# violetdenim/c3dgs

Hardware: AMD Instinct MI355X
Metric: raster views/sec fwd+bwd @1920x1080 (higher is better)
Workload: dtype f32; 1 GPU; BASELINE.json configs[2]: synth-v1 3M Gaussians, SH deg 3, indexed-camera rasterizer (QAT inner loop), mark_visible+fwd+bwd, 1 view/step/GPU; gaussians=3000000, width=1920, height=1080, sh_codebook=304096, gaussian_codebook=754096, parallelism=replicas x1

## Files before the change

__graft_entry__.py:

```python
import os
import subprocess
import sys

ROOT = os.path.dirname(os.path.abspath(__file__))
if ROOT not in sys.path:
    sys.path.insert(0, ROOT)


def build() -> None:
    from c3dgs_amd import build as hip_build
    lib = hip_build.build()
    assert os.path.exists(lib)
    for variant in hip_build.VARIANTS:
        assert os.path.exists(hip_build.build_variant(variant))
    subprocess.check_call(["make", "-C", os.path.join(ROOT, "oracle"), "-s"])
    import c3dgs_amd
    from c3dgs_amd import _lib
    L = _lib.lib()
    assert L.c3dgs_abi_version() == 4


def smoke() -> None:
    import numpy as np
    import torch
    from tests import cases, gpu_util, synth
    from oracle import oracle as orc

    assert torch.cuda.is_available(), "smoke() needs a GPU"
    torch.cuda.set_device(0)
    for name in ("base", "indexed"):
        inp, cam, indexed = cases.make_case(name)
        st = cases.oracle_forward(inp, cam)
        fw = gpu_util.hip_forward(inp, cam, indexed)
        u = gpu_util.unpack(fw)
        np.testing.assert_array_equal(u["radii"], st.radii)
        np.testing.assert_array_equal(u["keys_sorted"], st.keys_sorted)
        np.testing.assert_array_equal(u["point_list"], st.point_list)
        assert gpu_util.psnr(u["out_color"], st.out_color) >= 80.0
        dL = synth.grad_image(cam["W"], cam["H"]).numpy()
        ref = orc.rasterize_backward(st, dL)
        got = gpu_util.hip_backward(fw, dL)
        for k, v in got.items():
            if ref[k].shape == v.shape and v.size:
                err = gpu_util.rel_inf(v, ref[k])
                assert err <= 1e-4, (name, k, err)
    import c3dgs_amd
    g = torch.Generator().manual_seed(0)
    x = (torch.randn(4096, 48, generator=g) * 0.1).float()
    cb = (torch.randn(512, 48, generator=g) * 0.1).float()
    d, i = c3dgs_amd.weightedDistance(x.cuda(), cb.cuda())
    d_ref, i_ref = orc.weighted_distance(x.numpy(), cb.numpy())
    np.testing.assert_array_equal(i.cpu().numpy(), i_ref)
    np.testing.assert_array_equal(d.cpu().numpy().view(np.uint32), d_ref.view(np.uint32))
    print("smoke ok")


if __name__ == "__main__":
    build()
    if "--smoke" in sys.argv:
        smoke()
```

c3dgs_amd/build.py:

```python
import os
import subprocess
import sys
from concurrent.futures import ThreadPoolExecutor

HERE = os.path.dirname(os.path.abspath(__file__))
CSRC = os.path.join(HERE, "csrc")
OBJ = os.path.join(HERE, "build")
LIB = os.path.join(HERE, "libc3dgs_hip.so")
HIPCC = os.environ.get("HIPCC", "/opt/rocm/bin/hipcc")
ARCH = "gfx950"

COMMON = ["--offload-arch=" + ARCH, "-O3", "-fPIC", "-std=c++17", "-Wall", "-Wno-unused-function",
          "-fno-gpu-rdc", "-DNDEBUG"]
SOURCES = {
    "c_abi.hip": [],
    "c_abi_debug.hip": [],
    "preprocess.hip": ["-ffp-contract=off"],
    "backward_preprocess.hip": ["-ffp-contract=off"] + os.environ.get("C3DGS_BWDPRE_FLAGS", "").split(),
    "binning.hip": [],
    "radix_sort.hip": os.environ.get("C3DGS_SORT_FLAGS", "").split(),
    "render.hip": os.environ.get("C3DGS_RENDER_FLAGS", "-fno-slp-vectorize").split(),
    "vq.hip": ["-mllvm", "-amdgpu-mfma-vgpr-form"] + os.environ.get("C3DGS_VQ_FLAGS", "").split(),
    "draws.hip": [],
    "loss.hip": [],
    "metrics.hip": [],
    "encode.hip": [],
    "knn.hip": ["-ffp-contract=off"],
    "adam.hip": ["-ffp-contract=off"],
    "qat.hip": ["-ffp-contract=off"],
    "densify.hip": ["-ffp-contract=off"],
}
HEADERS = [os.path.join(CSRC, "common.hpp"), os.path.join(CSRC, "gsmath.hpp"), os.path.join(CSRC, "render_diag.hpp"),
           os.path.join(HERE, "..", "include", "c3dgs_hip.h"), os.path.join(HERE, "..", "include", "c3dgs_hip_debug.h")]


def _stale(target, deps):
    if not os.path.exists(target):
        return True
    t = os.path.getmtime(target)
    return any(os.path.getmtime(d) > t for d in deps)


def _compile(name, extra, verbose):
    src = os.path.join(CSRC, name)
    obj = os.path.join(OBJ, name.replace(".hip", ".o"))
    cmd = [HIPCC] + COMMON + extra + ["-c", src, "-o", obj]
    if verbose:
        print(" ".join(cmd), flush=True)
    subprocess.check_call(cmd)
    return obj


VARIANTS = {"spin1": {"radix_sort.hip": ["-DC3DGS_OS_SPIN_LIMIT=1u"]}}
def _diag(mode):
    return {src: ["-DC3DGS_DIAG", mode] for src in ("render.hip", "radix_sort.hip", "diag.hip")}


DIAG_VARIANTS = {"lanes": _diag("-DC3DGS_COUNT_LANES"), "bwdtime": _diag("-DC3DGS_BWD_TIMING"), "ostime": _diag("-DC3DGS_OS_TIMING")}


def build_variant(name, verbose=False):
    build(verbose=verbose)
    flags = {**VARIANTS, **DIAG_VARIANTS}[name]
    odir = os.path.join(HERE, "build", "variant_" + name)
    os.makedirs(odir, exist_ok=True)
    lib = os.path.join(HERE, f"libc3dgs_hip_{name}.so")
    objs, rebuilt = [], False
    for src in list(SOURCES) + [f for f in flags if f not in SOURCES]:
        extra = SOURCES.get(src, [])
        obj = os.path.join(OBJ, src.replace(".hip", ".o"))
        if src in flags:
            obj = os.path.join(odir, src.replace(".hip", ".o"))
            if _stale(obj, [os.path.join(CSRC, src)] + HEADERS + [os.path.abspath(__file__)]):
                cmd = [HIPCC] + COMMON + extra + flags[src] + ["-c", os.path.join(CSRC, src), "-o", obj]
                if verbose:
                    print(" ".join(cmd), flush=True)
                subprocess.check_call(cmd)
                rebuilt = True
        objs.append(obj)
    if rebuilt or _stale(lib, objs):
        subprocess.check_call([HIPCC, "--offload-arch=" + ARCH, "-shared", "-fPIC", "-o", lib] + objs)
    return lib


def build(force=False, verbose=False):
    os.makedirs(OBJ, exist_ok=True)
    deps_common = HEADERS + [os.path.abspath(__file__)]
    todo, objs = [], []
    for name, extra in SOURCES.items():
        obj = os.path.join(OBJ, name.replace(".hip", ".o"))
        objs.append(obj)
        if force or _stale(obj, [os.path.join(CSRC, name)] + deps_common):
            todo.append((name, extra))
    if todo:
        with ThreadPoolExecutor(max_workers=min(4, len(todo))) as ex:
            list(ex.map(lambda t: _compile(t[0], t[1], verbose), todo))
    if force or todo or _stale(LIB, objs):
        cmd = [HIPCC, "--offload-arch=" + ARCH, "-shared", "-fPIC", "-o", LIB] + objs
        if verbose:
            print(" ".join(cmd), flush=True)
        subprocess.check_call(cmd)
    return LIB


if __name__ == "__main__":
    print(build(force="--force" in sys.argv, verbose="--verbose" in sys.argv or "-v" in sys.argv))
    for flag, table in (("--variants", VARIANTS), ("--diag", DIAG_VARIANTS)):
        for v in table if flag in sys.argv else ():
            print(build_variant(v, verbose="--verbose" in sys.argv or "-v" in sys.argv))
```

c3dgs_amd/csrc/binning.hip:

```cpp
#include "common.hpp"
#include <rocprim/device/device_radix_sort.hpp>
#include <rocprim/iterator/counting_iterator.hpp>

namespace c3dgs {

size_t scan_temp_bytes(int P)
{
    size_t a = 0, b = 0;
    (void)rocprim::radix_sort_pairs(nullptr, b, (const uint32_t*)nullptr, (uint32_t*)nullptr, (const uint32_t*)nullptr,
                                    (uint32_t*)nullptr, (size_t)P, 0u, 32u);
    size_t m = a > b ? a : b;
    const size_t os = onesweep_depth_temp_bytes(P);
    if (os > m) m = os;
    return m < 256 ? 256 : m;
}

size_t sort_temp_bytes(int R, int end_bit, int key_bytes)
{
    size_t bytes = 0;
    if (key_bytes == 4)
        (void)rocprim::radix_sort_pairs(nullptr, bytes, (const uint32_t*)nullptr, (uint32_t*)nullptr,
                                        (const uint32_t*)nullptr, (uint32_t*)nullptr, (size_t)R, 0u, (unsigned)end_bit);
    else
        (void)rocprim::radix_sort_pairs(nullptr, bytes, (const uint16_t*)nullptr, (uint16_t*)nullptr,
                                        (const uint32_t*)nullptr, (uint32_t*)nullptr, (size_t)R, 0u, (unsigned)end_bit);
    const size_t os = onesweep_tile_temp_bytes(R, end_bit, key_bytes);
    if (os > bytes) bytes = os;
    const size_t reuse = compact_bin_layout(R).bin_bytes;
    if (reuse > bytes) bytes = reuse;
    return bytes < 256 ? 256 : bytes;
}

__global__ void __launch_bounds__(256)
gather_u64_kernel(int n, const uint32_t* __restrict__ idx, const uint2* __restrict__ src, uint2* __restrict__ dst)
{
    const int i = blockIdx.x * 256 + threadIdx.x;
    if (i < n) dst[i] = src[idx[i]];
}

size_t depth_sort_clear_bytes(int P)
{
    return (onesweep_enabled() && (size_t)P < ((size_t)1 << 30)) ? onesweep_depth_clear_bytes(P) : 0;
}
size_t tile_sort_clear_bytes(int R, int end_bit, int key_bytes)
{
    return (onesweep_enabled() && (size_t)R < ((size_t)1 << 30)) ? onesweep_tile_clear_bytes(R, end_bit, key_bytes) : 0;
}

hipError_t run_depth_sort(void* temp, size_t temp_bytes, const uint32_t* kin, uint32_t* kout, const uint32_t* vin,
                          uint32_t* vout, int P, const uint2* rects, uint2* rects_sorted, hipStream_t s, bool ctrl_cleared,
                          bool rects_fit_bytes)
{
    if (onesweep_enabled() && (size_t)P < ((size_t)1 << 30))
        return onesweep_depth_sort(temp, temp_bytes, kin, kout, vin, vout, P, rects, rects_sorted, s, ctrl_cleared, rects_fit_bytes);
    hipError_t e = vin ? rocprim::radix_sort_pairs(temp, temp_bytes, kin, kout, vin, vout, (size_t)P, 0u, 32u, s)
                       : rocprim::radix_sort_pairs(temp, temp_bytes, kin, kout, rocprim::counting_iterator<uint32_t>(0u), vout,
                                                   (size_t)P, 0u, 32u, s);
    if (e != hipSuccess) return e;
    gather_u64_kernel<<<(P + 255) / 256, 256, 0, s>>>(P, vout, rects, rects_sorted);
    return hipGetLastError();
}

hipError_t run_tile_sort(void* temp, size_t temp_bytes, const void* kin, void* kout, int key_bytes, const uint32_t* vin,
                         uint32_t* vout, int R, int end_bit, hipStream_t s, bool ctrl_cleared)
{
    if (key_bytes == 4) {
        if (onesweep_enabled() && (size_t)R < ((size_t)1 << 30))
            return onesweep_tile_sort32(temp, temp_bytes, (const uint32_t*)kin, (uint32_t*)kout, vin, vout, R, end_bit, s, ctrl_cleared);
        return rocprim::radix_sort_pairs(temp, temp_bytes, (const uint32_t*)kin, (uint32_t*)kout, vin, vout, (size_t)R, 0u, (unsigned)end_bit, s);
    }
    if (onesweep_enabled() && (size_t)R < ((size_t)1 << 30))
        return onesweep_tile_sort(temp, temp_bytes, (const uint16_t*)kin, (uint16_t*)kout, vin, vout, R, end_bit, s, ctrl_cleared);
    return rocprim::radix_sort_pairs(temp, temp_bytes, (const uint16_t*)kin, (uint16_t*)kout, vin, vout, (size_t)R, 0u, (unsigned)end_bit, s);
}

}
```

c3dgs_amd/csrc/c_abi.hip:

```cpp
#include "common.hpp"
#include <cstdlib>
#include <cstring>
#include <mutex>
#include <vector>

namespace c3dgs {

static thread_local std::string g_last_error;
void set_error(const std::string& msg) { g_last_error = msg; }

#define C3DGS_STAGE_TABLE(X)                                                                                                   \
    X(MARK_VISIBLE, "mark_visible") X(PREPROCESS, "preprocess") X(DEPTH_SORT, "depth_sort") X(SCAN, "scan")                    \
    X(DUPLICATE, "duplicate_with_keys") X(SORT, "sort") X(RANGES, "identify_ranges") X(RENDER_FWD, "render_forward")           \
    X(ZERO_PARTIALS, "zero_partials") X(RENDER_BWD, "render_backward") X(BWD_PREPROCESS, "backward_preprocess")                \
    X(WDIST, "weighted_distance") X(VQ_ACC, "vq_accumulate") X(VQ_APPLY, "vq_apply") X(LOSS_FWD, "l1_ssim_forward")            \
    X(LOSS_BWD, "l1_ssim_backward") X(QAT_OBSERVE, "qat_observe") X(QAT_CODEBOOKS, "qat_codebooks")                            \
    X(QAT_VISIBLE, "qat_visible") X(QAT_POINTS, "qat_points") X(QAT_POINTS_BWD, "qat_points_backward")                         \
    X(QAT_CODEBOOKS_BWD, "qat_codebooks_backward") X(ADAM, "adam_step") X(KNN_SORT, "knn_sort") X(KNN_BOUNDS, "knn_bounds")    \
    X(KNN_QUERY, "knn_query")
#define C3DGS_X(id, name) ST_##id,
enum Stage { C3DGS_STAGE_TABLE(C3DGS_X) ST_COUNT };
#undef C3DGS_X
#define C3DGS_X(id, name) name,
static const char* const kStageNames[ST_COUNT] = { C3DGS_STAGE_TABLE(C3DGS_X) };
#undef C3DGS_X
struct ProfRec { int stage; hipEvent_t a, b; };
static std::mutex g_prof_mu;
static bool g_prof_on = false;
static int g_prof_only = -1;
static std::vector<ProfRec> g_prof_recs;
static std::vector<hipEvent_t> g_prof_pool;

struct StageTimer {
    bool on; int stage; hipStream_t s; hipEvent_t a{}, b{};
    StageTimer(int stage_, hipStream_t s_) : on(g_prof_on && (g_prof_only < 0 || g_prof_only == stage_)), stage(stage_), s(s_)
    {
        if (!on) return;
        std::lock_guard<std::mutex> lk(g_prof_mu);
        auto get = [&](hipEvent_t& e) {
            if (!g_prof_pool.empty()) { e = g_prof_pool.back(); g_prof_pool.pop_back(); }
            else if (hipEventCreate(&e) != hipSuccess) on = false;
        };
        get(a); get(b);
        if (on) (void)hipEventRecord(a, s);
    }
    ~StageTimer()
    {
        if (!on) return;
        (void)hipEventRecord(b, s);
        std::lock_guard<std::mutex> lk(g_prof_mu);
        g_prof_recs.push_back({ stage, a, b });
    }
};
#define C3DGS_STAGE_CHECK(stage, debug, stream) C3DGS_STAGE(kStageNames[stage], debug, stream)
#define C3DGS_TIMED_STAGE(stage, debug, stream, ...)                                                \
    do {                                                                                            \
        { StageTimer t_(stage, stream); __VA_ARGS__; }                                              \
        C3DGS_STAGE_CHECK(stage, debug, stream);                                                    \
    } while (0)

struct HostRead {
    uint32_t* pinned = nullptr;
    uint32_t* dev = nullptr;
    uint32_t seq = 0;
    hipEvent_t ev{};
    HostRead()
    {
        const char* e = std::getenv("C3DGS_HOST_READ_COPY");
        const bool want_map = !(e && e[0] == '1');
        if (want_map && hipHostMalloc((void**)&pinned, 64, hipHostMallocMapped | hipHostMallocPortable | hipHostMallocCoherent) == hipSuccess) {
            void* d = nullptr;
            if (hipHostGetDevicePointer(&d, pinned, 0) == hipSuccess) dev = (uint32_t*)d;
            std::memset(pinned, 0, 64);
        } else {
            (void)hipGetLastError();
            if (hipHostMalloc((void**)&pinned, 64, hipHostMallocDefault) != hipSuccess) { pinned = nullptr; return; }
        }
        if (hipEventCreateWithFlags(&ev, hipEventDisableTiming) != hipSuccess) { (void)hipHostFree(pinned); pinned = nullptr; dev = nullptr; }
    }
    uint32_t begin()
    {
        if (!dev) return 0u;
        if (++seq == 0u) seq = 1u;
        return seq;
    }
    int copy_words(const uint32_t* src, hipStream_t s)
    {
        C3DGS_HIP_TRY(hipMemcpyAsync(pinned, src, 2 * sizeof(uint32_t), hipMemcpyDeviceToHost, s));
        return C3DGS_OK;
    }
    int queue_copy(const uint32_t* src, hipStream_t s)
    {
        if (dev) return C3DGS_OK;
        if (int rc = copy_words(src, s)) return rc;
        C3DGS_HIP_TRY(hipEventRecord(ev, s));
        return C3DGS_OK;
    }
    int wait(const uint32_t* src, hipStream_t s, uint32_t words[2])
    {
        if (dev) {
            volatile uint32_t* pad = pinned;
            bool seen = false;
            for (long spins = 0; !seen; spins++) {
                seen = __atomic_load_n(&pad[2], __ATOMIC_ACQUIRE) == seq;
                if (!seen && (spins & 0xffff) == 0xffff) {
                    const hipError_t q = hipStreamQuery(s);
                    if (q == hipErrorNotReady) continue;
                    if (q != hipSuccess) return fail(C3DGS_E_HIP, std::string("num_rendered read: ") + hipGetErrorString(q));
                    seen = __atomic_load_n(&pad[2], __ATOMIC_ACQUIRE) == seq;
                    if (!seen) {
                        if (int rc = copy_words(src, s)) return rc;
                        C3DGS_HIP_TRY(hipStreamSynchronize(s));
                        seen = true;
                    }
                }
            }
        } else {
            hipError_t q = hipErrorNotReady;
            for (long spins = 0; spins < 20000000L && (q = hipEventQuery(ev)) == hipErrorNotReady; spins++) { }
            if (q == hipErrorNotReady) q = hipEventSynchronize(ev);
            if (q != hipSuccess) return fail(C3DGS_E_HIP, std::string("num_rendered read: ") + hipGetErrorString(q));
        }
        words[0] = pinned[0]; words[1] = pinned[1];
        return C3DGS_OK;
    }
};
static HostRead& host_read()
{
    static thread_local HostRead h;
    return h;
}

static int validate(const c3dgs_raster_params* p, bool indexed, bool is_backward)
{
    if (!p) return fail(C3DGS_E_INVALID, "params is NULL");
    if (p->P < 0 || p->W <= 0 || p->H <= 0) return fail(C3DGS_E_INVALID, "P, W, H must be non-negative / positive");
    if (p->P == 0) return C3DGS_OK;
    if (!p->means3D) return fail(C3DGS_E_INVALID, "means3D must have dimensions (num_points, 3)");
    if (!p->background || !p->viewmatrix || !p->projmatrix || !p->campos)
        return fail(C3DGS_E_INVALID, "background, viewmatrix, projmatrix and campos are required");
    if (!is_backward && !p->opacities)
        return fail(C3DGS_E_INVALID, "opacities is required");
    if ((p->sh == nullptr) == (p->colors_precomp == nullptr))
        return fail(C3DGS_E_INVALID, "Please provide excatly one of either SHs or precomputed colors!");
    const bool has_sr = p->scales != nullptr && p->rotations != nullptr;
    if ((p->scales != nullptr) != (p->rotations != nullptr) || has_sr == (p->cov3D_precomp != nullptr))
        return fail(C3DGS_E_INVALID, "Please provide exactly one of either scale/rotation pair or precomputed 3D covariance!");
    if (p->sh) {
        if (p->D < 0 || p->D > 3) return fail(C3DGS_E_INVALID, "SH degree must be in [0,3]");
        if (p->M < (p->D + 1) * (p->D + 1)) return fail(C3DGS_E_INVALID, "sh has fewer coefficients than the active degree needs");
    }
    if (indexed) {
        if (p->sh && !p->sh_indices) return fail(C3DGS_E_INVALID, "indexed rasterizer: sh_indices is required with sh");
        if (has_sr && (!p->g_indices || !p->scale_factors))
            return fail(C3DGS_E_INVALID, "indexed rasterizer: g_indices and scale_factors are required with scales/rotations");
    } else if (p->sh_indices || p->g_indices || p->scale_factors) {
        return fail(C3DGS_E_INVALID, "non-indexed rasterizer: sh_indices / g_indices / scale_factors must be NULL");
    }
    if (tiles_x(p->W) > 65535 || tiles_y(p->H) > 65535) return fail(C3DGS_E_INVALID, "image too large for 16-bit tile coordinates");
    if ((unsigned long long)tiles_x(p->W) * tiles_x(p->W) * tiles_y(p->H) >= (1ull << 32))
        return fail(C3DGS_E_INVALID, "image too large: (tiles per row)^2 x (tile rows) must stay below 2^32");
    return C3DGS_OK;
}

static int forward_impl(const c3dgs_raster_params* pp, bool indexed, c3dgs_resize_fn geom_resize, void* geom_user,
                        c3dgs_resize_fn binning_resize, void* binning_user, c3dgs_resize_fn image_resize, void* image_user,
                        float* out_color, int32_t* radii, int32_t* num_rendered, void* stream_)
{
    if (int rc = validate(pp, indexed, false)) return rc;
    if (!out_color || !num_rendered) return fail(C3DGS_E_INVALID, "out_color and num_rendered are required");
    if (!geom_resize || !binning_resize || !image_resize) return fail(C3DGS_E_INVALID, "resize callbacks are required");
    c3dgs_raster_params p = *pp;
    if (!indexed) { p.sh_indices = nullptr; p.g_indices = nullptr; p.scale_factors = nullptr; }
    hipStream_t s = (hipStream_t)stream_;
    const int P = p.P, W = p.W, H = p.H;
    const int gx = tiles_x(W), gy = tiles_y(H);
    *num_rendered = 0;

    ImageLayout IL; image_layout(W, H, &IL);
    void* img_base = image_resize(image_user, IL.total_bytes);
    if (!img_base) return fail(C3DGS_E_ALLOC, "image buffer allocation failed");
    const ImgPtrs img = img_ptrs(img_base, W, H);

    if (P == 0) {
        C3DGS_HIP_TRY(hipMemsetAsync(out_color, 0, (size_t)3 * W * H * sizeof(float), s));
        C3DGS_HIP_TRY(hipMemsetAsync(img_base, 0, IL.total_bytes, s));
        return C3DGS_OK;
    }
    if (!radii) return fail(C3DGS_E_INVALID, "radii is required");

    c3dgs_geom_layout GL; geom_layout(P, &GL);
    void* geom_base = geom_resize(geom_user, GL.total_bytes + geom_gtab_bytes(p));
    if (!geom_base) return fail(C3DGS_E_ALLOC, "geometry buffer allocation failed");
    const GeomPtrs g = geom_ptrs(geom_base, P);

    uint32_t* sort_err = onesweep_error_word();
    if (!sort_err) return fail(C3DGS_E_HIP, "cannot resolve the sort error word");
    HostRead& hr = host_read();
    if (!hr.pinned) return fail(C3DGS_E_HIP, "pinned host buffer allocation failed");
    const uint32_t host_seq = hr.begin();
    const size_t dclear = depth_sort_clear_bytes(P) <= g.scan_temp_bytes ? depth_sort_clear_bytes(P) : 0;
    { StageTimer t_(ST_PREPROCESS, s);
      if (geom_gtab_bytes(p)) launch_pack_codebook(p, g.gtab, s);
      launch_preprocess(p, g, radii, img.ranges, sort_err, g.scan_temp, dclear / 16, hr.dev, host_seq, s); }
    C3DGS_STAGE_CHECK(ST_PREPROCESS, p.debug, s);
    const uint32_t* r_words = g.block_base + (P + 255) / 256;
    if (int rc = hr.queue_copy(r_words, s)) return rc;
    { StageTimer t_(ST_DEPTH_SORT, s);
      C3DGS_HIP_TRY(run_depth_sort(g.scan_temp, g.scan_temp_bytes, g.depth_keys, g.depth_keys_sorted, nullptr, g.depth_order, P,
                                   reinterpret_cast<const uint2*>(g.rects), g.sorted_offsets, s, dclear != 0,
                                   gx <= 255 && gy <= 255)); }
    C3DGS_STAGE_CHECK(ST_DEPTH_SORT, p.debug, s);
    if (p.debug && onesweep_timed_out(s)) return fail(C3DGS_E_HIP, "depth sort: look-back timed out");
    C3DGS_TIMED_STAGE(ST_SCAN, p.debug, s, launch_depth_order_scan(P, g, s));
    uint32_t words[2];
    if (int rc = hr.wait(r_words, s, words)) return rc;
    const uint32_t R_u = words[0];
    if (words[1] != 0) {
        C3DGS_HIP_TRY(hipMemsetAsync(sort_err, 0, sizeof(uint32_t), s));
        return fail(C3DGS_E_HIP, "radix sort look-back timed out in an earlier rasterizer call on this device: that call's "
                                 "image is NaN and its gradients are invalid (flag cleared, this call was not run)");
    }
    if (R_u > 0x7fffffffu) return fail(C3DGS_E_INVALID, "num_rendered overflows int32");
    const int R = (int)R_u;
    *num_rendered = R;

    c3dgs_binning_layout BL; binning_layout(R, W, H, &BL);
    void* bin_base = binning_resize(binning_user, BL.total_bytes);
    if (!bin_base) return fail(C3DGS_E_ALLOC, "binning buffer allocation failed");
    const BinPtrs b = bin_ptrs(bin_base, R, W, H);

    if (R > 0) {
        const int end_bit = tile_sort_end_bit(W, H);
        size_t tclear = tile_sort_clear_bytes(R, end_bit, b.key_bytes);
        if (tclear > b.sort_temp_bytes) tclear = 0;
        C3DGS_TIMED_STAGE(ST_DUPLICATE, p.debug, s, launch_duplicate_with_keys(P, g, b, gx, sort_err, b.sort_temp, tclear / 16, s));
        { StageTimer t_(ST_SORT, s);
          C3DGS_HIP_TRY(run_tile_sort(b.sort_temp, b.sort_temp_bytes, b.keys_unsorted, b.keys_sorted, b.key_bytes, b.values_unsorted,
                                      b.point_list, R, end_bit, s, tclear != 0)); }
        C3DGS_STAGE_CHECK(ST_SORT, p.debug, s);
        if (p.debug && onesweep_timed_out(s)) return fail(C3DGS_E_HIP, "tile sort: look-back timed out");
        C3DGS_TIMED_STAGE(ST_RANGES, p.debug, s, launch_identify_ranges(R, b.keys_sorted, b.key_bytes, img.ranges, sort_err, s));
    }
    C3DGS_TIMED_STAGE(ST_RENDER_FWD, p.debug, s,
                      launch_render_forward(W, H, img, b.point_list, g.splat, p.background, out_color, compact_ptrs(b, R), sort_err, s));
    return C3DGS_OK;
}

static int backward_impl(const c3dgs_raster_params* pp, bool indexed, const int32_t* radii, const void* geom_buffer,
                         const void* binning_buffer, const void* image_buffer, int32_t R, const float* dL_dout_color,
                         c3dgs_resize_fn ws_resize, void* ws_user, const c3dgs_raster_grads* grads, void* stream_)
{
    if (int rc = validate(pp, indexed, true)) return rc;
    if (!grads) return fail(C3DGS_E_INVALID, "grads is NULL");
    c3dgs_raster_params p = *pp;
    if (!indexed) { p.sh_indices = nullptr; p.g_indices = nullptr; p.scale_factors = nullptr; }
    hipStream_t s = (hipStream_t)stream_;
    const int P = p.P, W = p.W, H = p.H;

    void* cb_zero = nullptr;
    size_t cb_zero16 = 0;
    if (indexed) {
        const size_t n_sh = (grads->dL_dsh && p.sh) ? (size_t)p.SHS * p.M * 3 * sizeof(float) : 0;
        const size_t n_rot = (grads->dL_drotations && p.scales) ? (size_t)p.GS * 4 * sizeof(float) : 0;
        const size_t n_sc = (grads->dL_dscales && p.scales) ? (size_t)p.GS * 3 * sizeof(float) : 0;
        char* a_sh = (char*)grads->dL_dsh; char* a_rot = (char*)grads->dL_drotations; char* a_sc = (char*)grads->dL_dscales;
        if (n_sh && n_rot && n_sc && a_rot == a_sh + n_sh && a_sc == a_rot + n_rot) {
            const size_t n = n_sh + n_rot + n_sc;
            if (p.P > 0 && R >= 0 && ((uintptr_t)a_sh & 15u) == 0) {
                cb_zero = a_sh; cb_zero16 = n / 16;
                if (n % 16) C3DGS_HIP_TRY(hipMemsetAsync(a_sh + cb_zero16 * 16, 0, n % 16, s));
            } else {
                C3DGS_HIP_TRY(hipMemsetAsync(a_sh, 0, n, s));
            }
        } else {
            if (n_sh) C3DGS_HIP_TRY(hipMemsetAsync(a_sh, 0, n_sh, s));
            if (n_sc) C3DGS_HIP_TRY(hipMemsetAsync(a_sc, 0, n_sc, s));
            if (n_rot) C3DGS_HIP_TRY(hipMemsetAsync(a_rot, 0, n_rot, s));
        }
    }
    if (P == 0) return C3DGS_OK;
    if (!radii || !geom_buffer || !image_buffer || !dL_dout_color || (R > 0 && !binning_buffer))
        return fail(C3DGS_E_INVALID, "radii, forward buffers and dL_dout_color are required");
    if (!ws_resize) return fail(C3DGS_E_INVALID, "workspace callback is required");
    if (R < 0) return fail(C3DGS_E_INVALID, "R must be >= 0");

    const GeomPtrs g = geom_ptrs(const_cast<void*>(geom_buffer), P);
    const ImgPtrs img = img_ptrs(const_cast<void*>(image_buffer), W, H);
    void* ws_base = ws_resize(ws_user, c3dgs_backward_workspace_bytes(P, R));
    if (!ws_base) return fail(C3DGS_E_ALLOC, "backward workspace allocation failed");
    const BwdPtrs w = bwd_ptrs(ws_base, P, R);

    { StageTimer t_(ST_ZERO_PARTIALS, s);
      launch_backward_prep(R > 0 ? W : 0, H, img, w.touched, w.touched_bytes / 16, R > 0 ? nullptr : cb_zero, R > 0 ? 0 : cb_zero16, s); }
    if (R > 0) {
        const BinPtrs b = bin_ptrs(const_cast<void*>(binning_buffer), R, W, H);
        C3DGS_TIMED_STAGE(ST_RENDER_BWD, p.debug, s,
                          launch_render_backward(W, H, img, g.splat, g.block_base, p.background, dL_dout_color, w.partials, w.touched,
                                                 compact_ptrs(b, R), cb_zero, cb_zero16, s));
    }
    C3DGS_TIMED_STAGE(ST_BWD_PREPROCESS, p.debug, s, launch_backward_preprocess(p, radii, g, w, *grads, s));
    return C3DGS_OK;
}

}

using namespace c3dgs;

extern "C" {

const char* c3dgs_last_error(void) { return g_last_error.c_str(); }

int c3dgs_profile_enable(int on)
{
    std::lock_guard<std::mutex> lk(g_prof_mu);
    g_prof_on = on != 0;
    return C3DGS_OK;
}

int c3dgs_profile_only(const char* stage_name)
{
    std::lock_guard<std::mutex> lk(g_prof_mu);
    g_prof_only = -1;
    if (!stage_name || !*stage_name) return C3DGS_OK;
    for (int i = 0; i < ST_COUNT; i++)
        if (std::strcmp(stage_name, kStageNames[i]) == 0) { g_prof_only = i; return C3DGS_OK; }
    return fail(C3DGS_E_INVALID, std::string("profile_only: unknown stage ") + stage_name);
}

int c3dgs_profile_read(c3dgs_stage_time* out, int capacity)
{
    std::vector<ProfRec> recs;
    {
        std::lock_guard<std::mutex> lk(g_prof_mu);
        recs.swap(g_prof_recs);
    }
    double total[ST_COUNT] = { 0 };
    long long count[ST_COUNT] = { 0 };
    for (auto& r : recs) {
        float ms = 0.f;
        if (hipEventSynchronize(r.b) == hipSuccess && hipEventElapsedTime(&ms, r.a, r.b) == hipSuccess) {
            total[r.stage] += (double)ms;
            count[r.stage]++;
        }
    }
    {
        std::lock_guard<std::mutex> lk(g_prof_mu);
        for (auto& r : recs) { g_prof_pool.push_back(r.a); g_prof_pool.push_back(r.b); }
    }
    int n = 0;
    for (int i = 0; i < ST_COUNT && n < capacity; i++) {
        if (!count[i]) continue;
        std::memset(&out[n], 0, sizeof(out[n]));
        std::strncpy(out[n].name, kStageNames[i], sizeof(out[n].name) - 1);
        out[n].total_ms = total[i];
        out[n].count = count[i];
        n++;
    }
    return n;
}
int c3dgs_abi_version(void) { return C3DGS_ABI_VERSION; }

int c3dgs_get_geom_layout(int32_t P, c3dgs_geom_layout* out)
{
    if (!out || P < 0) return fail(C3DGS_E_INVALID, "bad arguments");
    geom_layout(P, out);
    return C3DGS_OK;
}
int c3dgs_get_binning_layout(int32_t R, int32_t W, int32_t H, c3dgs_binning_layout* out)
{
    if (!out || R < 0 || W <= 0 || H <= 0) return fail(C3DGS_E_INVALID, "bad arguments");
    binning_layout(R, W, H, out);
    return C3DGS_OK;
}
int c3dgs_get_image_layout(int32_t W, int32_t H, c3dgs_image_layout* out)
{
    if (!out || W <= 0 || H <= 0) return fail(C3DGS_E_INVALID, "bad arguments");
    ImageLayout L; image_layout(W, H, &L);
    *out = L;
    return C3DGS_OK;
}
int c3dgs_get_compact_layout(int32_t R, int32_t W, int32_t H, c3dgs_compact_layout* out)
{
    if (!out || R < 0 || W <= 0 || H <= 0) return fail(C3DGS_E_INVALID, "bad arguments");
    c3dgs_binning_layout BL; binning_layout(R, W, H, &BL);
    const CompactBinLayout C = compact_bin_layout(R);
    ImageLayout IL; image_layout(W, H, &IL);
    out->cqm = BL.sort_temp + C.cqm; out->cid = BL.sort_temp + C.cid;
    out->tile_used_c = IL.tile_used_c; out->n_contrib_c = IL.n_contrib_c;
    return C3DGS_OK;
}
int c3dgs_get_backward_layout(int32_t P, int32_t R, c3dgs_backward_layout* out)
{
    if (!out || P < 0 || R < 0) return fail(C3DGS_E_INVALID, "bad arguments");
    backward_layout(P, R, out);
    return C3DGS_OK;
}
size_t c3dgs_backward_workspace_bytes(int32_t P, int32_t R)
{
    c3dgs_backward_layout L; backward_layout(P, R, &L);
    return L.total_bytes;
}

int c3dgs_mark_visible(int32_t P, const float* means3D, const float* viewmatrix, const float* projmatrix, uint8_t* present,
                       void* stream)
{
    (void)projmatrix;
    if (P < 0) return fail(C3DGS_E_INVALID, "P must be >= 0");
    if (P == 0) return C3DGS_OK;
    if (!means3D || !viewmatrix || !present) return fail(C3DGS_E_INVALID, "means3D, viewmatrix and present are required");
    C3DGS_TIMED_STAGE(ST_MARK_VISIBLE, 0, (hipStream_t)stream, launch_mark_visible(P, means3D, viewmatrix, present, (hipStream_t)stream));
    return C3DGS_OK;
}

int c3dgs_mark_visible_pose(int32_t P, const float* means3D, const float* extrinsic_vector, uint8_t* present, void* stream)
{
    if (P < 0) return fail(C3DGS_E_INVALID, "P must be >= 0");
    if (P == 0) return C3DGS_OK;
    if (!means3D || !extrinsic_vector || !present) return fail(C3DGS_E_INVALID, "means3D, extrinsic_vector and present are required");
    C3DGS_TIMED_STAGE(ST_MARK_VISIBLE, 0, (hipStream_t)stream, launch_mark_visible_pose(P, means3D, extrinsic_vector, present, (hipStream_t)stream));
    return C3DGS_OK;
}

int c3dgs_camera_from_pose(const float* extrinsic_vector, float inv_tan_half_fovx, float inv_tan_half_fovy, float* viewmatrix,
                           float* projmatrix, float* campos, void* stream)
{
    if (!extrinsic_vector || !viewmatrix || !projmatrix || !campos) return fail(C3DGS_E_INVALID, "camera_from_pose: NULL pointer");
    launch_camera_from_pose(extrinsic_vector, inv_tan_half_fovx, inv_tan_half_fovy, viewmatrix, projmatrix, campos, (hipStream_t)stream);
    C3DGS_STAGE("camera_from_pose", 0, (hipStream_t)stream);
    return C3DGS_OK;
}

int c3dgs_rasterize_gaussians(const c3dgs_raster_params* p, c3dgs_resize_fn geom_resize, void* geom_user,
                              c3dgs_resize_fn binning_resize, void* binning_user, c3dgs_resize_fn image_resize,
                              void* image_user, float* out_color, int32_t* radii, int32_t* num_rendered, void* stream)
{
    return forward_impl(p, false, geom_resize, geom_user, binning_resize, binning_user, image_resize, image_user, out_color,
                        radii, num_rendered, stream);
}

int c3dgs_rasterize_gaussians_indexed(const c3dgs_raster_params* p, c3dgs_resize_fn geom_resize, void* geom_user,
                                      c3dgs_resize_fn binning_resize, void* binning_user, c3dgs_resize_fn image_resize,
                                      void* image_user, float* out_color, int32_t* radii, int32_t* num_rendered, void* stream)
{
    return forward_impl(p, true, geom_resize, geom_user, binning_resize, binning_user, image_resize, image_user, out_color,
                        radii, num_rendered, stream);
}

int c3dgs_rasterize_gaussians_backward(const c3dgs_raster_params* p, const int32_t* radii, const void* geom_buffer,
                                       const void* binning_buffer, const void* image_buffer, int32_t R,
                                       const float* dL_dout_color, c3dgs_resize_fn workspace_resize, void* workspace_user,
                                       const c3dgs_raster_grads* grads, void* stream)
{
    return backward_impl(p, false, radii, geom_buffer, binning_buffer, image_buffer, R, dL_dout_color, workspace_resize,
                         workspace_user, grads, stream);
}

int c3dgs_rasterize_gaussians_backward_indexed(const c3dgs_raster_params* p, const int32_t* radii, const void* geom_buffer,
                                               const void* binning_buffer, const void* image_buffer, int32_t R,
                                               const float* dL_dout_color, c3dgs_resize_fn workspace_resize,
                                               void* workspace_user, const c3dgs_raster_grads* grads, void* stream)
{
    return backward_impl(p, true, radii, geom_buffer, binning_buffer, image_buffer, R, dL_dout_color, workspace_resize,
                         workspace_user, grads, stream);
}

int c3dgs_weighted_distance(int64_t N, int32_t C, int32_t K, const float* coefs, const int64_t* gather,
                            const float* codebook, float* out_dist, int64_t* out_idx, void* stream)
{
    if (N < 0 || C < 0 || K <= 0) return fail(C3DGS_E_INVALID, "coefs and codebook must have same number of channels");
    if (N == 0) return C3DGS_OK;
    if (!coefs || !codebook || !out_dist || !out_idx) return fail(C3DGS_E_INVALID, "ceofs and codebook must have dimension 2");
    {
        StageTimer t_(ST_WDIST, (hipStream_t)stream);
        if (launch_weighted_distance(N, C, K, coefs, gather, codebook, out_dist, out_idx, (hipStream_t)stream))
            return fail(C3DGS_E_INVALID, "unsupported channel count");
    }
    C3DGS_STAGE_CHECK(ST_WDIST, 0, (hipStream_t)stream);
    return C3DGS_OK;
}

size_t c3dgs_weighted_distance_ws_bytes(int64_t N, int32_t C, int32_t K) { return wd_ws_bytes(N, C, K); }

int c3dgs_weighted_distance_ws(int64_t N, int32_t C, int32_t K, const float* coefs, const int64_t* gather, const float* codebook,
                               float* out_dist, int64_t* out_idx, void* ws, size_t ws_bytes, void* stream)
{
    if (N < 0 || C < 0 || K <= 0) return fail(C3DGS_E_INVALID, "coefs and codebook must have same number of channels");
    if (N == 0) return C3DGS_OK;
    if (!coefs || !codebook || !out_dist || !out_idx) return fail(C3DGS_E_INVALID, "ceofs and codebook must have dimension 2");
    {
        StageTimer t_(ST_WDIST, (hipStream_t)stream);
        if (launch_weighted_distance(N, C, K, coefs, gather, codebook, out_dist, out_idx, (hipStream_t)stream, ws, ws ? ws_bytes : 0))
            return fail(C3DGS_E_INVALID, "unsupported channel count");
    }
    C3DGS_STAGE_CHECK(ST_WDIST, 0, (hipStream_t)stream);
    return C3DGS_OK;
}

int c3dgs_vq_accumulate(int64_t B, int32_t K, int32_t D, const float* x, const float* w, const int64_t* gather,
                        const int64_t* idx, const float* dist, float* S, double* dist_sum, void* stream)
{
    if (B < 0 || K <= 0 || D <= 0) return fail(C3DGS_E_INVALID, "bad sizes");
    if (B == 0) return C3DGS_OK;
    if (!x || !w || !idx || !S) return fail(C3DGS_E_INVALID, "x, w, idx and S are required");
    C3DGS_TIMED_STAGE(ST_VQ_ACC, 0, (hipStream_t)stream, launch_vq_accumulate(B, K, D, x, w, gather, idx, dist, S, dist_sum, (hipStream_t)stream));
    return C3DGS_OK;
}

int c3dgs_vq_sums(int64_t B, int32_t K, int32_t D, const float* x, const float* w, const int64_t* gather,
                  const float* codebook, float* dist, int64_t* idx, float* S, double* dist_sum, void* ws, size_t ws_bytes,
                  void* stream)
{
    if (B < 0 || K <= 0 || D <= 0) return fail(C3DGS_E_INVALID, "bad sizes");
    if (!S || !dist_sum) return fail(C3DGS_E_INVALID, "S and dist_sum are required");
    C3DGS_HIP_TRY(hipMemsetAsync(S, 0, (size_t)K * (D + 1) * sizeof(float), (hipStream_t)stream));
    C3DGS_HIP_TRY(hipMemsetAsync(dist_sum, 0, sizeof(double), (hipStream_t)stream));
    if (B == 0) return C3DGS_OK;
    if (!x || !w || !codebook || !dist || !idx) return fail(C3DGS_E_INVALID, "x, w, codebook, dist and idx are required");
    {
        StageTimer t_(ST_WDIST, (hipStream_t)stream);
        if (launch_weighted_distance(B, K, D, x, gather, codebook, dist, idx, (hipStream_t)stream, ws, ws ? ws_bytes : 0))
            return fail(C3DGS_E_INVALID, "unsupported channel count");
    }
    C3DGS_STAGE_CHECK(ST_WDIST, 0, (hipStream_t)stream);
    return c3dgs_vq_accumulate(B, K, D, x, w, gather, idx, dist, S, dist_sum, stream);
}

int c3dgs_vq_step_supported(int32_t K, int32_t D, const float* x, const float* codebook, const void* ws, size_t ws_bytes)
{
    return (K > 0 && D > 0 && wd_presplit_supported(K, D, x, codebook, ws, ws_bytes)) ? 1 : 0;
}

int c3dgs_vq_step_sums(int32_t step, int64_t B, int32_t K, int32_t D, const float* x, const float* w, const int64_t* gather,
                       const float* codebook, float* dist, int64_t* idx, float* S, double* dist_sum, void* ws, size_t ws_bytes,
                       void* stream)
{
    hipStream_t s = (hipStream_t)stream;
    if (step < 0 || B <= 0 || K <= 0 || D <= 0) return fail(C3DGS_E_INVALID, "vq_step_sums: bad sizes");
    if (!x || !w || !codebook || !dist || !idx || !S || !dist_sum) return fail(C3DGS_E_INVALID, "vq_step_sums: NULL argument");
    if (!wd_presplit_supported(K, D, x, codebook, ws, ws_bytes))
        return fail(C3DGS_E_INVALID, "vq_step_sums: shape / scratch not served by the fused step (see c3dgs_vq_step_supported)");
    if (step == 0) {
        C3DGS_HIP_TRY(hipMemsetAsync(S, 0, (size_t)K * (D + 1) * sizeof(float), s));
        C3DGS_HIP_TRY(hipMemsetAsync(dist_sum, 0, sizeof(double), s));
    }
    {
        StageTimer t_(ST_WDIST, s);
        if (launch_weighted_distance(B, K, D, x, gather, codebook, dist, idx, s, ws, ws_bytes, step == 0 ? -1 : (step & 1)))
            return fail(C3DGS_E_INVALID, "vq_step_sums: unsupported shape");
        if (step == 0) launch_vq_seed_words(K, D, ws, s);
    }
    C3DGS_STAGE_CHECK(ST_WDIST, 0, s);
    C3DGS_TIMED_STAGE(ST_VQ_ACC, 0, s,
                      launch_vq_accumulate(B, K, D, x, w, gather, idx, dist, S, dist_sum, s, vq_next_absmax_word(K, D, ws, step & 1)));
    return C3DGS_OK;
}

int c3dgs_vq_step_apply(int32_t step, int32_t K, int32_t D, float* S, float* codebook, float* entry_importance, float decay,
                        float alpha, float eps, int32_t scale_normalize, void* ws, size_t ws_bytes, void* stream)
{
    if (step < 0 || K <= 0 || D <= 0 || !S || !codebook || !entry_importance) return fail(C3DGS_E_INVALID, "vq_step_apply: bad arguments");
    { StageTimer t_(ST_VQ_APPLY, (hipStream_t)stream);
      if (launch_vq_apply_split(K, D, S, codebook, entry_importance, decay, alpha, eps, scale_normalize, ws, ws_bytes, step & 1, (hipStream_t)stream))
          return fail(C3DGS_E_INVALID, "vq_step_apply: shape / scratch not served by the fused step (see c3dgs_vq_step_supported)"); }
    C3DGS_STAGE_CHECK(ST_VQ_APPLY, 0, (hipStream_t)stream);
    return C3DGS_OK;
}

int c3dgs_vq_apply(int32_t K, int32_t D, const float* S, float* codebook, float* entry_importance, float decay,
                   float alpha, float eps, int32_t scale_normalize, void* stream)
{
    if (K <= 0 || D <= 0 || !S || !codebook || !entry_importance) return fail(C3DGS_E_INVALID, "bad arguments");
    C3DGS_TIMED_STAGE(ST_VQ_APPLY, 0, (hipStream_t)stream,
                      launch_vq_apply(K, D, S, codebook, entry_importance, decay, alpha, eps, scale_normalize, (hipStream_t)stream));
    return C3DGS_OK;
}

size_t c3dgs_morton_workspace_bytes(int32_t P) { return morton_workspace_bytes(P); }

int c3dgs_morton_order(int32_t P, const float* xyz, int64_t* codes, int64_t* order, void* workspace, void* stream)
{
    if (P < 0) return fail(C3DGS_E_INVALID, "P must be >= 0");
    if (P == 0) return C3DGS_OK;
    if (!xyz || !codes || !order || !workspace) return fail(C3DGS_E_INVALID, "morton_order: bad arguments");
    if (run_morton_order(P, xyz, codes, order, workspace, (hipStream_t)stream)) return fail(C3DGS_E_HIP, "morton_order failed");
    C3DGS_STAGE("morton_order", 0, (hipStream_t)stream);
    return C3DGS_OK;
}

size_t c3dgs_knn_workspace_bytes(int32_t P) { return knn_workspace_bytes(P); }

int c3dgs_knn_mean_dist2(int32_t P, const float* xyz, float* out, void* workspace, void* stream)
{
    if (P < 0) return fail(C3DGS_E_INVALID, "knn_mean_dist2: P must be >= 0");
    if (P == 0) return C3DGS_OK;
    if (!xyz || !out || !workspace) return fail(C3DGS_E_INVALID, "knn_mean_dist2: bad arguments");
    hipStream_t s = (hipStream_t)stream;
    { StageTimer t_(ST_KNN_SORT, s);
      if (run_knn_sort(P, xyz, workspace, s)) return fail(C3DGS_E_HIP, "knn_mean_dist2: sort failed"); }
    C3DGS_STAGE_CHECK(ST_KNN_SORT, 0, s);
    C3DGS_TIMED_STAGE(ST_KNN_BOUNDS, 0, s, launch_knn_bounds(P, workspace, s));
    C3DGS_TIMED_STAGE(ST_KNN_QUERY, 0, s, launch_knn_query(P, workspace, out, s));
    return C3DGS_OK;
}

int c3dgs_abs_accumulate(int64_t n, const float* g, float* acc, void* stream)
{
    if (n < 0 || (n > 0 && (!g || !acc))) return fail(C3DGS_E_INVALID, "abs_accumulate: bad arguments");
    launch_abs_accumulate(n, g, acc, (hipStream_t)stream);
    C3DGS_STAGE("abs_accumulate", 0, (hipStream_t)stream);
    return C3DGS_OK;
}

int c3dgs_adam_step(int32_t n_tensors, const c3dgs_adam_tensor* tensors, double beta1, double beta2, double eps, void* stream)
{
    if (n_tensors < 0 || n_tensors > C3DGS_ADAM_MAX_TENSORS) return fail(C3DGS_E_INVALID, "adam_step: between 0 and 16 tensors per call");
    if (n_tensors == 0) return C3DGS_OK;
    if (!tensors) return fail(C3DGS_E_INVALID, "adam_step: tensors is NULL");
    for (int k = 0; k < n_tensors; k++)
        if (tensors[k].n > 0 && (!tensors[k].param || !tensors[k].grad || !tensors[k].exp_avg || !tensors[k].exp_avg_sq))
            return fail(C3DGS_E_INVALID, "adam_step: NULL tensor pointer");
    C3DGS_TIMED_STAGE(ST_ADAM, 0, (hipStream_t)stream, launch_adam(n_tensors, tensors, beta1, beta2, eps, (hipStream_t)stream));
    return C3DGS_OK;
}

static const int kRowsMaxCopies = 250;

int c3dgs_densify_classify(int32_t P, const float* accum, const float* denom, const float* scale_clone, const float* scale_split,
                           const float* scale_prune_self, const float* scale_prune_child, const float* opacity, float max_grad,
                           float dense_extent, float min_opacity, float big_extent, uint8_t* code, void* stream)
{
    if (P < 0) return fail(C3DGS_E_INVALID, "densify_classify: P must be >= 0");
    if (!(max_grad > 0.f)) return fail(C3DGS_E_INVALID, "densify_classify: max_grad must be > 0 (see include/c3dgs_hip.h)");
    if (P == 0) return C3DGS_OK;
    if (!accum || !denom || !scale_clone || !scale_split || !opacity || !code)
        return fail(C3DGS_E_INVALID, "densify_classify: NULL buffer");
    if ((scale_prune_self == nullptr) != (scale_prune_child == nullptr))
        return fail(C3DGS_E_INVALID, "densify_classify: scale_prune_self and scale_prune_child go together");
    launch_densify_classify(P, accum, denom, scale_clone, scale_split, scale_prune_self, scale_prune_child, opacity, max_grad,
                            dense_extent, min_opacity, big_extent, code, (hipStream_t)stream);
    C3DGS_STAGE("densify_classify", 0, (hipStream_t)stream);
    return C3DGS_OK;
}

size_t c3dgs_rows_plan_workspace_bytes(int32_t P) { return rows_plan_workspace_bytes(P); }

int c3dgs_rows_plan(int32_t P, const uint8_t* code, int32_t N, int64_t capacity, int32_t* src, uint8_t* kind, int32_t* draw_row,
                    int32_t* totals, void* workspace, void* stream)
{
    if (P < 0) return fail(C3DGS_E_INVALID, "rows_plan: P must be >= 0");
    if (N < 1 || N > kRowsMaxCopies) return fail(C3DGS_E_INVALID, "rows_plan: N must be between 1 and 250");
    if (capacity < 0) return fail(C3DGS_E_INVALID, "rows_plan: capacity must be >= 0");
    if ((int64_t)P * (2 + N) >= ((int64_t)1 << 31)) return fail(C3DGS_E_INVALID, "rows_plan: P * (2 + N) must fit 31 bits");
    if (!totals) return fail(C3DGS_E_INVALID, "rows_plan: totals is required");
    hipStream_t s = (hipStream_t)stream;
    if (P == 0) { C3DGS_HIP_TRY(hipMemsetAsync(totals, 0, 4 * sizeof(int32_t), s)); return C3DGS_OK; }
    if (!code || !workspace) return fail(C3DGS_E_INVALID, "rows_plan: NULL buffer");
    if (src && (!kind || !draw_row)) return fail(C3DGS_E_INVALID, "rows_plan: src, kind and draw_row go together");
    C3DGS_HIP_TRY(run_rows_plan(P, code, N, capacity, src, kind, draw_row, totals, workspace, s));
    C3DGS_STAGE("rows_plan", 0, s);
    return C3DGS_OK;
}

int c3dgs_rows_apply(int32_t P, int64_t P_new, const int32_t* src, const uint8_t* kind, const int32_t* draw_row, int32_t n_tensors,
                     const c3dgs_rows_tensor* tensors, int32_t N, int64_t n_draws, const float* rotation_raw, const float* std,
                     const float* z, int32_t log_scaling, int32_t half_xyz, void* stream)
{
    if (P < 0 || P_new < 0 || n_draws < 0) return fail(C3DGS_E_INVALID, "rows_apply: sizes must be >= 0");
    if (N < 1 || N > kRowsMaxCopies) return fail(C3DGS_E_INVALID, "rows_apply: N must be between 1 and 250");
    if (n_tensors < 0 || n_tensors > C3DGS_ROWS_MAX_TENSORS) return fail(C3DGS_E_INVALID, "rows_apply: between 0 and 16 tensors per call");
    if (P_new >= ((int64_t)1 << 31)) return fail(C3DGS_E_INVALID, "rows_apply: P_new must fit 31 bits");
    if (P_new == 0 || n_tensors == 0) return C3DGS_OK;
    if (P == 0) return fail(C3DGS_E_INVALID, "rows_apply: P_new > 0 rows cannot come from P = 0");
    if (!src || !kind || !draw_row || !tensors) return fail(C3DGS_E_INVALID, "rows_apply: NULL buffer");
    for (int k = 0; k < n_tensors; k++) {
        const c3dgs_rows_tensor& t = tensors[k];
        if (t.row_floats < 1 || t.row_floats > 4096) return fail(C3DGS_E_INVALID, "rows_apply: row_floats must be between 1 and 4096");
        if (!t.in_param || !t.out_param) return fail(C3DGS_E_INVALID, "rows_apply: NULL tensor pointer");
        const int nm = (t.in_exp_avg != nullptr) + (t.in_exp_avg_sq != nullptr) + (t.out_exp_avg != nullptr) + (t.out_exp_avg_sq != nullptr);
        if (nm != 0 && nm != 4) return fail(C3DGS_E_INVALID, "rows_apply: the four moment pointers go together");
        if (t.role != C3DGS_ROLE_COPY && t.role != C3DGS_ROLE_XYZ && t.role != C3DGS_ROLE_SCALING)
            return fail(C3DGS_E_INVALID, "rows_apply: unknown role");
        if (t.role != C3DGS_ROLE_COPY && t.row_floats != 3) return fail(C3DGS_E_INVALID, "rows_apply: xyz / scaling rows have 3 floats");
        if (t.role != C3DGS_ROLE_COPY && n_draws > 0 && (!std || !z || (t.role == C3DGS_ROLE_XYZ && !rotation_raw)))
            return fail(C3DGS_E_INVALID, "rows_apply: children need rotation_raw, std and z");
    }
    launch_rows_apply(P, P_new, src, kind, draw_row, n_tensors, tensors, N, n_draws, rotation_raw, std, z, log_scaling, half_xyz, (hipStream_t)stream);
    C3DGS_STAGE("rows_apply", 0, (hipStream_t)stream);
    return C3DGS_OK;
}

int c3dgs_densify_stats(int32_t P, const float* grad, const uint8_t* filter, const int32_t* radii, float* accum, float* denom,
                        float* max_radii, void* stream)
{
    if (P < 0) return fail(C3DGS_E_INVALID, "densify_stats: P must be >= 0");
    if (P == 0) return C3DGS_OK;
    if (!grad || !filter || !accum || !denom) return fail(C3DGS_E_INVALID, "densify_stats: NULL buffer");
    if ((radii == nullptr) != (max_radii == nullptr)) return fail(C3DGS_E_INVALID, "densify_stats: radii and max_radii go together");
    launch_densify_stats(P, grad, filter, radii, accum, denom, max_radii, (hipStream_t)stream);
    C3DGS_STAGE("densify_stats", 0, (hipStream_t)stream);
    return C3DGS_OK;
}

int c3dgs_extract_rot_scale(int32_t n, const float* cov6, float* rot, float* scale, void* stream)
{
    if (n < 0) return fail(C3DGS_E_INVALID, "extract_rot_scale: n must be >= 0");
    if (n == 0) return C3DGS_OK;
    if (!cov6 || !rot || !scale || (reinterpret_cast<uintptr_t>(rot) & 15)) return fail(C3DGS_E_INVALID, "extract_rot_scale: bad arguments");
    launch_extract_rot_scale(n, cov6, rot, scale, (hipStream_t)stream);
    C3DGS_STAGE("extract_rot_scale", 0, (hipStream_t)stream);
    return C3DGS_OK;
}

int c3dgs_l1_ssim_forward(int32_t C, int32_t H, int32_t W, const float* img, const float* gt, float* dmaps, double* sums,
                          void* stream)
{
    if (C <= 0 || H <= 0 || W <= 0 || !img || !gt || !sums) return fail(C3DGS_E_INVALID, "l1_ssim_forward: bad arguments");
    hipStream_t s = (hipStream_t)stream;
    C3DGS_HIP_TRY(hipMemsetAsync(sums, 0, 128 * sizeof(double), s));
    const size_t n = (size_t)C * H * W;
    C3DGS_TIMED_STAGE(ST_LOSS_FWD, 0, s,
                      launch_l1_ssim_forward(C, H, W, img, gt, dmaps, dmaps ? dmaps + n : nullptr, dmaps ? dmaps + 2 * n : nullptr, sums, s));
    return C3DGS_OK;
}

int c3dgs_l1_ssim_value(const double* sums, double l1_scale, double ssim_scale, double constant, float* out, void* stream)
{
    if (!sums || !out) return fail(C3DGS_E_INVALID, "l1_ssim_value: bad arguments");
    launch_l1_ssim_value(sums, l1_scale, ssim_scale, constant, out, (hipStream_t)stream);
    C3DGS_STAGE("l1_ssim_value", 0, (hipStream_t)stream);
    return C3DGS_OK;
}

int c3dgs_l1_ssim_backward(int32_t C, int32_t H, int32_t W, const float* img, const float* gt, const float* dmaps,
                           const float* grad_loss, float l1_coeff, float ssim_coeff, float* dL_dimg, void* stream)
{
    if (C <= 0 || H <= 0 || W <= 0 || !img || !gt || !dmaps || !grad_loss || !dL_dimg)
        return fail(C3DGS_E_INVALID, "l1_ssim_backward: bad arguments");
    hipStream_t s = (hipStream_t)stream;
    const size_t n = (size_t)C * H * W;
    C3DGS_TIMED_STAGE(ST_LOSS_BWD, 0, s,
                      launch_l1_ssim_backward(C, H, W, img, gt, dmaps, dmaps + n, dmaps + 2 * n, grad_loss, l1_coeff, ssim_coeff, dL_dimg, s));
    return C3DGS_OK;
}

size_t c3dgs_image_metrics_ws_bytes(int32_t N, int32_t C, int32_t H, int32_t W) { return image_metrics_ws_bytes(N, C, H, W); }

int c3dgs_image_metrics(int32_t N, int32_t C, int32_t H, int32_t W, const float* img, const float* gt, void* ws, size_t ws_bytes,
                        double* out, void* stream)
{
    if (N <= 0 || C <= 0 || H <= 0 || W <= 0) return fail(C3DGS_E_INVALID, "image_metrics: N, C, H and W must be positive");
    if (image_metrics_workgroups(N, C, H, W) > IMAGE_METRICS_MAX_WORKGROUPS)
        return fail(C3DGS_E_INVALID, "image_metrics: size overflow (N * C * H * W too large for one call; split the batch)");
    if (!img || !gt || !ws || !out) return fail(C3DGS_E_INVALID, "image_metrics: img, gt, ws and out are required");
    if (reinterpret_cast<uintptr_t>(ws) & 7) return fail(C3DGS_E_INVALID, "image_metrics: ws must be 8-byte aligned");
    const size_t need = image_metrics_ws_bytes(N, C, H, W);
    if (ws_bytes < need)
        return fail(C3DGS_E_INVALID, "image_metrics: ws too small (" + std::to_string(ws_bytes) + " bytes, need " +
                                         std::to_string(need) + ")");
    launch_image_metrics(N, C, H, W, img, gt, (double*)ws, out, (hipStream_t)stream);
    C3DGS_STAGE("image_metrics", 0, (hipStream_t)stream);
    return C3DGS_OK;
}

static int qat_validate(const c3dgs_qat_params* q, const char* who)
{
    if (!q) return fail(C3DGS_E_INVALID, std::string(who) + ": params is NULL");
    if (q->P < 0 || q->GS < 0 || q->SHS < 0 || q->M < 1) return fail(C3DGS_E_INVALID, std::string(who) + ": bad sizes");
    if (!q->state) return fail(C3DGS_E_INVALID, std::string(who) + ": state is required");
    if (q->features_dc && q->M > 1 && !q->features_rest)
        return fail(C3DGS_E_INVALID, std::string(who) + ": features_rest is required with features_dc when M > 1");
    if (reinterpret_cast<uintptr_t>(q->rotation) & 15) return fail(C3DGS_E_INVALID, std::string(who) + ": rotation must be 16-byte aligned");
    return C3DGS_OK;
}
static bool misaligned16(const void* p) { return (reinterpret_cast<uintptr_t>(p) & 15) != 0; }

size_t c3dgs_qat_workspace_bytes(void) { return qat_workspace_bytes(); }
size_t c3dgs_qat_scan_bytes(int32_t P) { return qat_scan_bytes(P); }

int c3dgs_qat_observe(const c3dgs_qat_params* q, void* workspace, void* stream)
{
    if (int rc = qat_validate(q, "qat_observe")) return rc;
    if (!workspace) return fail(C3DGS_E_INVALID, "qat_observe: workspace is required");
    C3DGS_TIMED_STAGE(ST_QAT_OBSERVE, 0, (hipStream_t)stream, launch_qat_observe(*q, workspace, (hipStream_t)stream));
    return C3DGS_OK;
}

int c3dgs_qat_codebooks(const c3dgs_qat_params* q, float* scales_n, float* rotations, float* shs, void* stream)
{
    if (int rc = qat_validate(q, "qat_codebooks")) return rc;
    if (misaligned16(rotations) || misaligned16(shs)) return fail(C3DGS_E_INVALID, "qat_codebooks: outputs must be 16-byte aligned");
    C3DGS_TIMED_STAGE(ST_QAT_CODEBOOKS, 0, (hipStream_t)stream, launch_qat_codebooks(*q, scales_n, rotations, shs, (hipStream_t)stream));
    return C3DGS_OK;
}

int c3dgs_qat_codebooks_backward(const c3dgs_qat_params* q, const float* dL_dscales_n, const float* dL_drotations,
                                 const float* dL_dshs, float* dL_dscaling, float* dL_drotation, float* dL_dfeatures_dc,
                                 float* dL_dfeatures_rest, void* stream)
{
    if (int rc = qat_validate(q, "qat_codebooks_backward")) return rc;
    if (misaligned16(dL_drotations) || misaligned16(dL_drotation) || misaligned16(dL_dshs))
        return fail(C3DGS_E_INVALID, "qat_codebooks_backward: rotation / sh gradients must be 16-byte aligned");
    if (dL_dshs && q->features_dc && (!dL_dfeatures_dc || (q->M > 1 && !dL_dfeatures_rest)))
        return fail(C3DGS_E_INVALID, "qat_codebooks_backward: dL_dfeatures_dc / dL_dfeatures_rest are required with dL_dshs");
    C3DGS_TIMED_STAGE(ST_QAT_CODEBOOKS_BWD, 0, (hipStream_t)stream,
                      launch_qat_codebooks_backward(*q, dL_dscales_n, dL_drotations, dL_dshs, dL_dscaling, dL_drotation, dL_dfeatures_dc,
                                                    dL_dfeatures_rest, (hipStream_t)stream));
    return C3DGS_OK;
}

int c3dgs_qat_visible(const c3dgs_qat_params* q, const float* viewmatrix, uint8_t* visible, int32_t* rank, int32_t* count,
                      void* scan_workspace, void* stream)
{
    if (int rc = qat_validate(q, "qat_visible")) return rc;
    if (!count) return fail(C3DGS_E_INVALID, "qat_visible: count is required");
    hipStream_t s = (hipStream_t)stream;
    if (q->P == 0) { C3DGS_HIP_TRY(hipMemsetAsync(count, 0, sizeof(int32_t), s)); return C3DGS_OK; }
    if (!q->xyz || !viewmatrix || !visible || !rank || !scan_workspace) return fail(C3DGS_E_INVALID, "qat_visible: bad arguments");
    { StageTimer t_(ST_QAT_VISIBLE, s); C3DGS_HIP_TRY(run_qat_visible(*q, viewmatrix, visible, rank, count, scan_workspace, s)); }
    C3DGS_STAGE_CHECK(ST_QAT_VISIBLE, 0, s);
    return C3DGS_OK;
}

int c3dgs_qat_points(const c3dgs_qat_params* q, const uint8_t* visible, const int32_t* rank, const int64_t* sh_indices,
                     const int64_t* g_indices, float* means3D, float* opacities, float* scale_factors, int64_t* sh_indices_out,
                     int64_t* g_indices_out, void* stream)
{
    if (int rc = qat_validate(q, "qat_points")) return rc;
    if ((visible == nullptr) != (rank == nullptr)) return fail(C3DGS_E_INVALID, "qat_points: visible and rank go together");
    C3DGS_TIMED_STAGE(ST_QAT_POINTS, 0, (hipStream_t)stream,
                      launch_qat_points(*q, visible, rank, sh_indices, g_indices, means3D, opacities, scale_factors, sh_indices_out,
                                        g_indices_out, (hipStream_t)stream));
    return C3DGS_OK;
}

int c3dgs_qat_points_backward(const c3dgs_qat_params* q, const uint8_t* visible, const int32_t* rank, const float* dL_dmeans3D,
                              const float* dL_dmeans2D, const float* dL_dopacities, const float* dL_dscale_factors,
                              float* dL_dxyz, float* dL_dscreenspace, float* dL_dopacity, float* dL_dscaling_factor, void* stream)
{
    if (int rc = qat_validate(q, "qat_points_backward")) return rc;
    if ((visible == nullptr) != (rank == nullptr)) return fail(C3DGS_E_INVALID, "qat_points_backward: visible and rank go together");
    if ((dL_dopacity && dL_dopacities && !q->opacity) || (dL_dscaling_factor && dL_dscale_factors && !q->scaling_factor))
        return fail(C3DGS_E_INVALID, "qat_points_backward: the raw opacity / scaling_factor are needed to recompute the masks");
    C3DGS_TIMED_STAGE(ST_QAT_POINTS_BWD, 0, (hipStream_t)stream,
                      launch_qat_points_backward(*q, visible, rank, dL_dmeans3D, dL_dmeans2D, dL_dopacities, dL_dscale_factors, dL_dxyz,
                                                 dL_dscreenspace, dL_dopacity, dL_dscaling_factor, (hipStream_t)stream));
    return C3DGS_OK;
}

int c3dgs_qat_quantize(const c3dgs_qat_params* q, int32_t scaling_is_exp, int8_t* opacity, int8_t* scaling, int8_t* scaling_factor,
                       int8_t* rotation, int8_t* features_dc, int8_t* features_rest, void* stream)
{
    if (int rc = qat_validate(q, "qat_quantize")) return rc;
    if (rotation && (reinterpret_cast<uintptr_t>(rotation) & 3)) return fail(C3DGS_E_INVALID, "qat_quantize: rotation output must be 4-byte aligned");
    launch_qat_quantize(*q, scaling_is_exp, opacity, scaling, scaling_factor, rotation, features_dc, features_rest, (hipStream_t)stream);
    C3DGS_STAGE("qat_quantize", 0, (hipStream_t)stream);
    return C3DGS_OK;
}

int c3dgs_fake_quantize(int64_t n, const float* x, c3dgs_fq_state* state, int32_t observe, int32_t enabled,
                        float averaging_constant, float* out, void* workspace, void* stream)
{
    if (n < 0) return fail(C3DGS_E_INVALID, "fake_quantize: n must be >= 0");
    if (n == 0) return C3DGS_OK;
    if (!x || !state || !out || (observe && !workspace)) return fail(C3DGS_E_INVALID, "fake_quantize: bad arguments");
    launch_fake_quantize(n, x, state, observe, enabled, averaging_constant, out, workspace, (hipStream_t)stream);
    C3DGS_STAGE("fake_quantize", 0, (hipStream_t)stream);
    return C3DGS_OK;
}

int c3dgs_fake_quantize_backward(int64_t n, const float* x, const c3dgs_fq_state* state, int32_t enabled, const float* g,
                                 float* dx, void* stream)
{
    if (n < 0) return fail(C3DGS_E_INVALID, "fake_quantize_backward: n must be >= 0");
    if (n == 0) return C3DGS_OK;
    if (!x || !state || !g || !dx) return fail(C3DGS_E_INVALID, "fake_quantize_backward: bad arguments");
    launch_fake_quantize_backward(n, x, state, enabled, g, dx, (hipStream_t)stream);
    C3DGS_STAGE("fake_quantize_backward", 0, (hipStream_t)stream);
    return C3DGS_OK;
}

}
```

c3dgs_amd/csrc/common.hpp:

```cpp
#pragma once
#include <hip/hip_runtime.h>
#include <cstdint>
#include <cstddef>
#include <cstdio>
#include <cstring>
#include <string>

#include "../../include/c3dgs_hip.h"

namespace c3dgs {

constexpr int TILE = 16;
constexpr int TILE_PIX = 256;
constexpr int SPLAT_F4 = 3;
constexpr int PARTIAL_FLOATS = 9;
constexpr int BWD_LIST = 1024;

void set_error(const std::string& msg);
inline int fail(int code, const std::string& msg) { set_error(msg); return code; }

#define C3DGS_HIP_TRY(expr)                                                                         \
    do {                                                                                            \
        hipError_t e__ = (expr);                                                                    \
        if (e__ != hipSuccess)                                                                      \
            return ::c3dgs::fail(C3DGS_E_HIP, std::string(#expr) + ": " + hipGetErrorString(e__));  \
    } while (0)

#define C3DGS_STAGE(name, debug, stream)                                                            \
    do {                                                                                            \
        hipError_t e__ = hipGetLastError();                                                         \
        if (e__ == hipSuccess && (debug)) e__ = hipStreamSynchronize(stream);                       \
        if (e__ != hipSuccess)                                                                      \
            return ::c3dgs::fail(C3DGS_E_HIP, std::string("stage ") + name + ": " + hipGetErrorString(e__)); \
    } while (0)

__device__ __forceinline__ uint32_t f2ord(float f)
{
    const uint32_t u = __float_as_uint(f);
    return (u & 0x80000000u) ? ~u : (u | 0x80000000u);
}
__device__ __host__ __forceinline__ float ord2f(uint32_t o)
{
    const uint32_t u = (o & 0x80000000u) ? (o & 0x7fffffffu) : ~o;
    float f;
    memcpy(&f, &u, 4);
    return f;
}

inline size_t align_up(size_t v, size_t a = 256) { return (v + a - 1) / a * a; }

size_t scan_temp_bytes(int P);
size_t sort_temp_bytes(int R, int end_bit, int key_bytes = 2);

inline int tiles_x(int W) { return (W + TILE - 1) / TILE; }
inline int tiles_y(int H) { return (H + TILE - 1) / TILE; }

inline uint32_t higher_msb(uint32_t n)
{
    uint32_t msb = sizeof(n) * 4, step = msb;
    while (step > 1) {
        step /= 2;
        if (n >> msb) msb += step; else msb -= step;
    }
    if (n >> msb) msb++;
    return msb;
}

inline void geom_layout(int P, c3dgs_geom_layout* L)
{
    size_t o = 0, p = (size_t)(P > 0 ? P : 1);
    L->splat = o;             o = align_up(o + p * SPLAT_F4 * 16);
    L->depth_keys = o;        o = align_up(o + p * 4);
    L->depth_keys_sorted = o; o = align_up(o + p * 4);
    L->depth_order = o;       o = align_up(o + p * 4);
    L->sorted_offsets = o;    o = align_up(o + p * 8);
    L->inst_offset = o;       o = align_up(o + p * 4);
    L->rects = o;             o = align_up(o + p * 8);
    L->clamped = o;           o = align_up(o + p);
    L->block_base = o;        o = align_up(o + ((p + 255) / 256 + 2) * 4);
    L->depth_base = o;        o = align_up(o + ((p + 255) / 256 + 1) * 4);
    L->scan_temp = o;         L->scan_temp_bytes = scan_temp_bytes((int)p);
    o = align_up(o + L->scan_temp_bytes);
    L->total_bytes = o;
}

inline size_t geom_gtab_bytes(const c3dgs_raster_params& p) { return (p.g_indices && p.scales) ? align_up((size_t)(p.GS > 0 ? p.GS : 1) * 32) : 0; }

inline int tile_key_bytes_for(long long T) { return T > 65536 ? 4 : 2; }
inline int tile_key_bytes(int W, int H) { return tile_key_bytes_for((long long)tiles_x(W) * tiles_y(H)); }
inline int tile_sort_end_bit_for(long long T)
{
    const int msb = (int)higher_msb((uint32_t)T), kbits = 8 * tile_key_bytes_for(T);
    return msb < kbits ? msb : kbits;
}
inline int tile_sort_end_bit(int W, int H) { return tile_sort_end_bit_for((long long)tiles_x(W) * tiles_y(H)); }

inline void binning_layout(int R, int W, int H, c3dgs_binning_layout* L)
{
    size_t o = 0, r = (size_t)(R > 0 ? R : 1);
    const int end_bit = tile_sort_end_bit(W, H);
    const size_t kb = (size_t)tile_key_bytes(W, H);
    L->keys_unsorted = o;   o = align_up(o + r * kb);
    L->values_unsorted = o; o = align_up(o + r * 4);
    L->keys_sorted = o;     o = align_up(o + r * kb);
    L->point_list = o;      o = align_up(o + r * 4);
    L->sort_temp = o;       L->sort_temp_bytes = sort_temp_bytes((int)r, end_bit, (int)kb);
    o = align_up(o + L->sort_temp_bytes);
    L->total_bytes = o;
}

struct ImageLayout : c3dgs_image_layout { size_t tile_used_c, n_contrib_c; };
inline void image_layout(int W, int H, ImageLayout* L)
{
    size_t o = 0, n = (size_t)W * H, t = (size_t)tiles_x(W) * tiles_y(H);
    L->final_T = o;     o = align_up(o + n * 4);
    L->n_contrib = o;   o = align_up(o + n * 4);
    L->ranges = o;      o = align_up(o + t * 8);
    L->tile_used = o;   o = align_up(o + t * 4);
    L->tile_order = o;  o = align_up(o + t * 4);
    L->tile_used_c = o; o = align_up(o + t * 4);
    L->n_contrib_c = o; o = align_up(o + n * 4);
    L->total_bytes = o;
}

struct CompactBinLayout { size_t cqm, cid, bin_bytes; };
inline CompactBinLayout compact_bin_layout(int R)
{
    const size_t r = (size_t)(R > 0 ? R : 1);
    CompactBinLayout C;
    C.cqm = 0; C.cid = align_up(r); C.bin_bytes = C.cid + align_up(r * 4);
    return C;
}

inline void backward_layout(int P, int R, c3dgs_backward_layout* L)
{
    size_t o = 0, r = (size_t)(R > 0 ? R : 1), n_lists = ((size_t)(P > 0 ? P : 1) + BWD_LIST - 1) / BWD_LIST;
    L->partials = o;   o = align_up(o + r * PARTIAL_FLOATS * sizeof(float));
    L->touched = o;    o = align_up(o + r);
    L->live_ids = o;   o = align_up(o + n_lists * BWD_LIST * 4);
    L->live_slots = o; o = align_up(o + n_lists * BWD_LIST * 4);
    L->live_count = o; o = align_up(o + n_lists * 4);
    L->list_len = BWD_LIST;
    L->total_bytes = o;
}

struct GeomPtrs {
    float4* splat; uint32_t* depth_keys; uint32_t* depth_keys_sorted;
    uint32_t* depth_order; uint2* sorted_offsets; uint32_t* inst_offset; uint16_t* rects;
    uint8_t* clamped; uint32_t* block_base; uint32_t* depth_base; void* scan_temp; size_t scan_temp_bytes;
    float4* gtab;
};
struct BinPtrs {
    void* keys_unsorted; uint32_t* values_unsorted; void* keys_sorted; uint32_t* point_list;
    void* sort_temp; size_t sort_temp_bytes; int key_bytes;
};
struct ImgPtrs { float* final_T; uint32_t* n_contrib; uint2* ranges; uint32_t* tile_used; uint32_t* tile_order;
                 uint32_t* tile_used_c; uint32_t* n_contrib_c; };
struct CompactPtrs { uint8_t* cqm; uint32_t* cid; };
struct BwdPtrs { float* partials; uint8_t* touched; size_t touched_bytes;
                 uint32_t* live_ids; uint32_t* live_slots; uint32_t* live_count; };

inline GeomPtrs geom_ptrs(void* base, int P)
{
    c3dgs_geom_layout L; geom_layout(P, &L);
    char* b = (char*)base;
    return { (float4*)(b + L.splat), (uint32_t*)(b + L.depth_keys), (uint32_t*)(b + L.depth_keys_sorted), (uint32_t*)(b + L.depth_order),
             (uint2*)(b + L.sorted_offsets), (uint32_t*)(b + L.inst_offset), (uint16_t*)(b + L.rects),
             (uint8_t*)(b + L.clamped), (uint32_t*)(b + L.block_base), (uint32_t*)(b + L.depth_base), (void*)(b + L.scan_temp),
             L.scan_temp_bytes, (float4*)(b + L.total_bytes) };
}
inline BinPtrs bin_ptrs(void* base, int R, int W, int H)
{
    c3dgs_binning_layout L; binning_layout(R, W, H, &L);
    char* b = (char*)base;
    return { (void*)(b + L.keys_unsorted), (uint32_t*)(b + L.values_unsorted), (void*)(b + L.keys_sorted),
             (uint32_t*)(b + L.point_list), (void*)(b + L.sort_temp), L.sort_temp_bytes, tile_key_bytes(W, H) };
}
inline ImgPtrs img_ptrs(void* base, int W, int H)
{
    ImageLayout L; image_layout(W, H, &L);
    char* b = (char*)base;
    return { (float*)(b + L.final_T), (uint32_t*)(b + L.n_contrib), (uint2*)(b + L.ranges), (uint32_t*)(b + L.tile_used),
             (uint32_t*)(b + L.tile_order), (uint32_t*)(b + L.tile_used_c), (uint32_t*)(b + L.n_contrib_c) };
}
inline CompactPtrs compact_ptrs(const BinPtrs& bp, int R)
{
    const CompactBinLayout C = compact_bin_layout(R);
    return { (uint8_t*)bp.sort_temp + C.cqm, (uint32_t*)((char*)bp.sort_temp + C.cid) };
}
inline BwdPtrs bwd_ptrs(void* base, int P, int R)
{
    c3dgs_backward_layout L; backward_layout(P, R, &L);
    char* b = (char*)base;
    return { (float*)(b + L.partials), (uint8_t*)(b + L.touched), L.live_ids - L.touched,
             (uint32_t*)(b + L.live_ids), (uint32_t*)(b + L.live_slots), (uint32_t*)(b + L.live_count) };
}

void launch_camera_from_pose(const float* pose, float inv_tan_x, float inv_tan_y, float* view, float* proj, float* campos, hipStream_t s);
void launch_mark_visible(int P, const float* means3D, const float* view, uint8_t* present, hipStream_t s);
void launch_mark_visible_pose(int P, const float* means3D, const float* pose7, uint8_t* present, hipStream_t s);
void launch_pack_codebook(const c3dgs_raster_params& p, float4* gtab, hipStream_t s);
void launch_preprocess(const c3dgs_raster_params& p, const GeomPtrs& g, int32_t* radii, uint2* ranges, const uint32_t* sort_err,
                       void* zero_span, size_t zero_n16, uint32_t* host_out, uint32_t host_seq, hipStream_t s);
void launch_depth_order_scan(int P, const GeomPtrs& g, hipStream_t s);
void launch_duplicate_with_keys(int P, const GeomPtrs& g, const BinPtrs& b, int grid_x, const uint32_t* sort_err,
                                void* zero_span, size_t zero_n16, hipStream_t s);
void launch_identify_ranges(int R, const void* keys_sorted, int key_bytes, uint2* ranges, const uint32_t* sort_err, hipStream_t s);
hipError_t run_depth_sort(void* temp, size_t temp_bytes, const uint32_t* kin, uint32_t* kout, const uint32_t* vin,
                          uint32_t* vout, int P, const uint2* rects, uint2* rects_sorted, hipStream_t s, bool ctrl_cleared = false,
                          bool rects_fit_bytes = false);
hipError_t run_tile_sort(void* temp, size_t temp_bytes, const void* kin, void* kout, int key_bytes, const uint32_t* vin,
                         uint32_t* vout, int R, int end_bit, hipStream_t s, bool ctrl_cleared = false);
size_t depth_sort_clear_bytes(int P);
size_t tile_sort_clear_bytes(int R, int end_bit, int key_bytes);
bool onesweep_enabled();
int onesweep_timed_out(hipStream_t s);
uint32_t* onesweep_error_word();
size_t onesweep_depth_temp_bytes(int P);
size_t onesweep_tile_temp_bytes(int R, int end_bit, int key_bytes = 2);
size_t onesweep_depth_clear_bytes(int P);
size_t onesweep_tile_clear_bytes(int R, int end_bit, int key_bytes);
hipError_t onesweep_depth_sort(void* temp, size_t temp_bytes, const uint32_t* kin, uint32_t* kout, const uint32_t* vin, uint32_t* vout,
                               int P, const uint2* gather_src, uint2* gather_dst, hipStream_t s, bool ctrl_cleared = false,
                               bool rects_fit_bytes = false);
hipError_t onesweep_tile_sort32(void* temp, size_t temp_bytes, const uint32_t* kin, uint32_t* kout, const uint32_t* vin, uint32_t* vout,
                                int R, int end_bit, hipStream_t s, bool ctrl_cleared = false);
hipError_t onesweep_tile_sort(void* temp, size_t temp_bytes, const uint16_t* kin, uint16_t* kout, const uint32_t* vin, uint32_t* vout,
                              int R, int end_bit, hipStream_t s, bool ctrl_cleared = false);
void launch_render_forward(int W, int H, const ImgPtrs& img, const uint32_t* point_list, const float4* splat,
                           const float* bg, float* out_color, const CompactPtrs& cl, const uint32_t* sort_err, hipStream_t s);
void launch_backward_prep(int W, int H, const ImgPtrs& img, void* zero_a, size_t n16_a, void* zero_b, size_t n16_b, hipStream_t s);
void launch_render_backward(int W, int H, const ImgPtrs& img, const float4* splat,
                            const uint32_t* block_base, const float* bg, const float* dL_dpix, float* partials,
                            uint8_t* touched, const CompactPtrs& cl, void* zero_span, size_t zero_n16, hipStream_t s);
void launch_backward_preprocess(const c3dgs_raster_params& p, const int32_t* radii, const GeomPtrs& g, const BwdPtrs& w,
                                const c3dgs_raster_grads& gr, hipStream_t s);
int launch_weighted_distance(int64_t N, int C, int K, const float* coefs, const int64_t* gather, const float* codebook,
                             float* out_dist, int64_t* out_idx, hipStream_t s, void* ws = nullptr, size_t ws_bytes = 0, int presplit = -1);
bool wd_presplit_supported(int C, int K, const float* coefs, const float* codebook, const void* ws, size_t ws_bytes);
int launch_vq_apply_split(int K, int D, float* S, float* codebook, float* entry_importance, float decay, float alpha, float eps,
                          int scale_normalize, void* ws, size_t ws_bytes, int parity, hipStream_t s);
void launch_vq_seed_words(int K, int D, void* ws, hipStream_t s);
uint32_t* vq_next_absmax_word(int K, int D, void* ws, int parity);
size_t wd_ws_bytes(int64_t N, int C, int K);
int launch_wd_debug_scores(int64_t N, int C, int K, const float* coefs, const float* codebook, float* scores, void* ws, size_t ws_bytes,
                           float* out_dist, int64_t* out_idx, hipStream_t s);
void launch_vq_accumulate(int64_t B, int K, int D, const float* x, const float* w, const int64_t* gather,
                          const int64_t* idx, const float* dist, float* S, double* dist_sum, hipStream_t s, uint32_t* clear_word = nullptr);
void launch_vq_apply(int K, int D, const float* S, float* codebook, float* entry_importance, float decay, float alpha,
                     float eps, int scale_normalize, hipStream_t s);

size_t morton_workspace_bytes(int P);
int run_morton_order(int P, const float* xyz, int64_t* codes_out, int64_t* order_out, void* workspace, hipStream_t s);
void launch_extract_rot_scale(int n, const float* cov6, float* rot, float* scale, hipStream_t s);
size_t knn_workspace_bytes(int P);
int run_knn_sort(int P, const float* xyz, void* workspace, hipStream_t s);
void launch_knn_bounds(int P, void* workspace, hipStream_t s);
void launch_knn_query(int P, const void* workspace, float* out, hipStream_t s);
void launch_adam(int n_tensors, const c3dgs_adam_tensor* tensors, double beta1, double beta2, double eps, hipStream_t s);
void launch_abs_accumulate(int64_t n, const float* g, float* acc, hipStream_t s);
void launch_densify_classify(int P, const float* accum, const float* denom, const float* scale_clone, const float* scale_split,
                             const float* scale_prune_self, const float* scale_prune_child, const float* opacity, float max_grad,
                             float dense_extent, float min_opacity, float big_extent, uint8_t* code, hipStream_t s);
size_t rows_plan_workspace_bytes(int P);
hipError_t run_rows_plan(int P, const uint8_t* code, int N, long long capacity, int32_t* src, uint8_t* kind, int32_t* draw_row,
                         int32_t* totals, void* workspace, hipStream_t s);
void launch_rows_apply(int P, long long P_new, const int32_t* src, const uint8_t* kind, const int32_t* draw_row, int n_tensors,
                       const c3dgs_rows_tensor* tensors, int N, long long n_draws, const float* rotation_raw, const float* std,
                       const float* z, int log_scaling, int half_xyz, hipStream_t s);
void launch_densify_stats(int P, const float* grad, const uint8_t* filter, const int32_t* radii, float* accum, float* denom,
                          float* max_radii, hipStream_t s);
void launch_l1_ssim_value(const double* sums, double l1_scale, double ssim_scale, double constant, float* out, hipStream_t s);
void launch_l1_ssim_forward(int C, int H, int W, const float* img, const float* gt, float* Dmu, float* Ds1, float* Ds12,
                            double* sums, hipStream_t s);
void launch_l1_ssim_backward(int C, int H, int W, const float* img, const float* gt, const float* Dmu, const float* Ds1,
                             const float* Ds12, const float* grad_loss, float l1_coeff, float ssim_coeff, float* dL_dimg,
                             hipStream_t s);
constexpr int64_t IMAGE_METRICS_MAX_WORKGROUPS = (int64_t(1) << 24) - 1;
int64_t image_metrics_workgroups(int N, int C, int H, int W);
size_t image_metrics_ws_bytes(int N, int C, int H, int W);
void launch_image_metrics(int N, int C, int H, int W, const float* img, const float* gt, double* partials, double* out,
                          hipStream_t s);

size_t qat_workspace_bytes();
size_t qat_scan_bytes(int P);
void launch_qat_observe(const c3dgs_qat_params& q, void* workspace, hipStream_t s);
void launch_qat_codebooks(const c3dgs_qat_params& q, float* scales_n, float* rotations, float* shs, hipStream_t s);
void launch_qat_codebooks_backward(const c3dgs_qat_params& q, const float* g_scales, const float* g_rot, const float* g_shs,
                                   float* d_scaling, float* d_rotation, float* d_dc, float* d_rest, hipStream_t s);
hipError_t run_qat_visible(const c3dgs_qat_params& q, const float* view, uint8_t* visible, int32_t* rank, int32_t* count,
                           void* scan_ws, hipStream_t s);
void launch_qat_points(const c3dgs_qat_params& q, const uint8_t* visible, const int32_t* rank, const int64_t* sh_idx,
                       const int64_t* g_idx, float* means3D, float* opac, float* sfac, int64_t* sh_out, int64_t* g_out,
                       hipStream_t s);
void launch_qat_points_backward(const c3dgs_qat_params& q, const uint8_t* visible, const int32_t* rank, const float* g_m3,
                                const float* g_m2, const float* g_op, const float* g_sf, float* d_xyz, float* d_screen,
                                float* d_op, float* d_sf, hipStream_t s);
void launch_qat_quantize(const c3dgs_qat_params& q, int scaling_exp, int8_t* opacity, int8_t* scaling, int8_t* scaling_factor,
                         int8_t* rotation, int8_t* features_dc, int8_t* features_rest, hipStream_t s);
void launch_fake_quantize(long long n, const float* x, c3dgs_fq_state* state, int observe, int enabled, float c, float* out,
                          void* workspace, hipStream_t s);
void launch_fake_quantize_backward(long long n, const float* x, const c3dgs_fq_state* state, int enabled, const float* g,
                                   float* dx, hipStream_t s);

}
```

c3dgs_amd/csrc/preprocess.hip:

```cpp
#include "common.hpp"
#include "gsmath.hpp"

namespace c3dgs {

template <bool POSE>
__global__ void __launch_bounds__(256)
mark_visible_kernel(int P, const float* __restrict__ means3D, const float* __restrict__ view_or_pose, uint8_t* __restrict__ present, int vec)
{
    const int j = blockIdx.x * 256 + threadIdx.x;
    const int i0 = 4 * j;
    if (i0 >= P) return;
    float vm[16];
    const float* view = view_or_pose;
    if (POSE) {
        const float x = view_or_pose[0], y = view_or_pose[1], z = view_or_pose[2], w = view_or_pose[3], tz = view_or_pose[6];
        const float d2 = y * y + z * z + x * x;
#pragma unroll
        for (int q = 0; q < 16; q++) vm[q] = 0.f;
        vm[2] = 2.0f * (x * z - w * y); vm[6] = 2.0f * (y * z + w * x); vm[10] = 1.0f + 2.0f * (z * z - d2); vm[14] = tz;
        view = vm;
    }
    if (vec && i0 + 4 <= P) {
        const float4* src = reinterpret_cast<const float4*>(means3D) + 3 * (size_t)j;
        const float4 a = src[0], b = src[1], c = src[2];
        const f3 p0 = { a.x, a.y, a.z }, p1 = { a.w, b.x, b.y }, p2 = { b.z, b.w, c.x }, p3 = { c.y, c.z, c.w };
        const uint32_t v0 = !(xform4x3(p0, view).z <= 0.01f), v1 = !(xform4x3(p1, view).z <= 0.01f);
        const uint32_t v2 = !(xform4x3(p2, view).z <= 0.01f), v3 = !(xform4x3(p3, view).z <= 0.01f);
        reinterpret_cast<uint32_t*>(present)[j] = v0 | (v1 << 8) | (v2 << 16) | (v3 << 24);
        return;
    }
    for (int i = i0; i < min(i0 + 4, P); i++) {
        f3 p = { means3D[3 * (size_t)i], means3D[3 * (size_t)i + 1], means3D[3 * (size_t)i + 2] };
        f3 pv = xform4x3(p, view);
        present[i] = !(pv.z <= 0.01f) ? 1 : 0;
    }
}

__global__ void __launch_bounds__(256)
pack_codebook_kernel(int GS, const float* __restrict__ scales, const float* __restrict__ rotations, float4* __restrict__ gtab)
{
    const int g = blockIdx.x * 256 + threadIdx.x;
    if (g >= GS) return;
    gtab[2 * (size_t)g] = *reinterpret_cast<const float4*>(rotations + 4 * (size_t)g);
    gtab[2 * (size_t)g + 1] = make_float4(scales[3 * (size_t)g], scales[3 * (size_t)g + 1], scales[3 * (size_t)g + 2], 0.f);
}

void launch_pack_codebook(const c3dgs_raster_params& p, float4* gtab, hipStream_t s)
{
    if (p.GS <= 0) return;
    pack_codebook_kernel<<<(p.GS + 255) / 256, 256, 0, s>>>(p.GS, p.scales, p.rotations, gtab);
}

void launch_mark_visible(int P, const float* means3D, const float* view, uint8_t* present, hipStream_t s)
{
    if (P <= 0) return;
    const int vec = ((reinterpret_cast<uintptr_t>(means3D) & 15u) == 0 && (reinterpret_cast<uintptr_t>(present) & 3u) == 0) ? 1 : 0;
    mark_visible_kernel<false><<<((P + 3) / 4 + 255) / 256, 256, 0, s>>>(P, means3D, view, present, vec);
}

void launch_mark_visible_pose(int P, const float* means3D, const float* pose, uint8_t* present, hipStream_t s)
{
    if (P <= 0) return;
    const int vec = ((reinterpret_cast<uintptr_t>(means3D) & 15u) == 0 && (reinterpret_cast<uintptr_t>(present) & 3u) == 0) ? 1 : 0;
    mark_visible_kernel<true><<<((P + 3) / 4 + 255) / 256, 256, 0, s>>>(P, means3D, pose, present, vec);
}

__global__ void camera_from_pose_kernel(const float* __restrict__ pose, float inv_tan_x, float inv_tan_y, float pa, float pb,
                                        float* __restrict__ view, float* __restrict__ proj, float* __restrict__ campos)
{
    if (threadIdx.x != 0 || blockIdx.x != 0) return;
    const float x = pose[0], y = pose[1], z = pose[2], w = pose[3], tx = pose[4], ty = pose[5], tz = pose[6];
    const float d2 = y * y + z * z + x * x;
    float M[4][4];
    M[0][0] = 1.0f + 2.0f * (x * x - d2); M[0][1] = 2.0f * (x * y - w * z);        M[0][2] = 2.0f * (x * z + w * y);        M[0][3] = tx;
    M[1][0] = 2.0f * (x * y + w * z);        M[1][1] = 1.0f + 2.0f * (y * y - d2); M[1][2] = 2.0f * (y * z - w * x);        M[1][3] = ty;
    M[2][0] = 2.0f * (x * z - w * y);        M[2][1] = 2.0f * (y * z + w * x);        M[2][2] = 1.0f + 2.0f * (z * z - d2); M[2][3] = tz;
    M[3][0] = 0.f; M[3][1] = 0.f; M[3][2] = 0.f; M[3][3] = 1.f;
#pragma unroll
    for (int i = 0; i < 4; i++) {
#pragma unroll
        for (int j = 0; j < 4; j++) view[i * 4 + j] = M[j][i];
        proj[i * 4 + 0] = M[0][i] * inv_tan_x;
        proj[i * 4 + 1] = M[1][i] * inv_tan_y;
        proj[i * 4 + 2] = M[2][i] * pa + M[3][i] * pb;
        proj[i * 4 + 3] = M[2][i];
    }
    const double a = M[0][0], b = M[0][1], c = M[0][2], d = M[1][0], e = M[1][1], f = M[1][2], g = M[2][0], h = M[2][1], k = M[2][2];
    const double A = e * k - f * h, B = -(d * k - f * g), C = d * h - e * g;
    const double det = a * A + b * B + c * C;
    const double inv[3][3] = { { A / det, -(b * k - c * h) / det, (b * f - c * e) / det },
                               { B / det, (a * k - c * g) / det, -(a * f - c * d) / det },
                               { C / det, -(a * h - b * g) / det, (a * e - b * d) / det } };
#pragma unroll
    for (int r = 0; r < 3; r++) campos[r] = (float)-(inv[r][0] * (double)tx + inv[r][1] * (double)ty + inv[r][2] * (double)tz);
}

void launch_camera_from_pose(const float* pose, float inv_tan_x, float inv_tan_y, float* view, float* proj, float* campos, hipStream_t s)
{
    const float pa = (float)(1.0 * 100.0 / (100.0 - 0.01)), pb = (float)(-(100.0 * 0.01) / (100.0 - 0.01));
    camera_from_pose_kernel<<<1, 64, 0, s>>>(pose, inv_tan_x, inv_tan_y, pa, pb, view, proj, campos);
}

template <int DEG>
__device__ __forceinline__ void sh_to_rgb(const float* c, float x, float y, float z, float out[3])
{
#pragma unroll
    for (int ch = 0; ch < 3; ch++) {
        float res = SH_C0 * c[0 * 3 + ch];
        if (DEG > 0) {
            res = res - SH_C1 * y * c[1 * 3 + ch] + SH_C1 * z * c[2 * 3 + ch] - SH_C1 * x * c[3 * 3 + ch];
            if (DEG > 1) {
                float xx = x * x, yy = y * y, zz = z * z;
                float xy = x * y, yz = y * z, xz = x * z;
                res = res + SH_C2_0 * xy * c[4 * 3 + ch] + SH_C2_1 * yz * c[5 * 3 + ch] +
                      SH_C2_2 * (2.0f * zz - xx - yy) * c[6 * 3 + ch] + SH_C2_3 * xz * c[7 * 3 + ch] +
                      SH_C2_4 * (xx - yy) * c[8 * 3 + ch];
                if (DEG > 2) {
                    res = res + SH_C3_0 * y * (3.0f * xx - yy) * c[9 * 3 + ch] + SH_C3_1 * xy * z * c[10 * 3 + ch] +
                          SH_C3_2 * y * (4.0f * zz - xx - yy) * c[11 * 3 + ch] +
                          SH_C3_3 * z * (2.0f * zz - 3.0f * xx - 3.0f * yy) * c[12 * 3 + ch] +
                          SH_C3_4 * x * (4.0f * zz - xx - yy) * c[13 * 3 + ch] + SH_C3_5 * z * (xx - yy) * c[14 * 3 + ch] +
                          SH_C3_6 * x * (xx - 3.0f * yy) * c[15 * 3 + ch];
                }
            }
        }
        out[ch] = res + 0.5f;
    }
}

struct PreArgs {
    int P, M, W, H, gx, gy;
    const float* means3D; const float* sh; const float* colors_precomp; const float* opacities;
    const float* scales; const float* scale_factors; const float* rotations; const float* cov3D_precomp;
    const int64_t* sh_indices; const int64_t* g_indices;
    const float* view; const float* proj; const float* campos;
    float tan_fovx, tan_fovy, focal_x, focal_y, scale_modifier;
    int prefiltered, clamp_color;
    int32_t* radii; float4* splat; uint16_t* rects; uint8_t* clamped;
    uint32_t* depth_keys;
    uint32_t* inst_offset; uint32_t* block_total;
    uint2* ranges; int T;
    const float4* gtab;
    uint4* zero_span; size_t zero_n16;
};

template <int DEG>
__global__ void __launch_bounds__(256) preprocess_kernel(const PreArgs a)
{
    __shared__ uint32_t s_wsum[4];
    const int t = threadIdx.x, lane = t & 63, wave = t >> 6;
    const int i = blockIdx.x * 256 + t;
    const bool in_range = i < a.P;
    for (int q = i; q < a.T; q += gridDim.x * 256) a.ranges[q] = make_uint2(0u, 0u);
    if (a.zero_n16) {
        const size_t per = (a.zero_n16 + gridDim.x - 1) / gridDim.x, z0 = (size_t)blockIdx.x * per, z1 = min(z0 + per, a.zero_n16);
        for (size_t q = z0 + t; q < z1; q += 256) a.zero_span[q] = make_uint4(0u, 0u, 0u, 0u);
    }

    int32_t out_radius = 0;
    uint32_t out_tiles = 0;
    uint32_t out_key = 0xffffffffu;
    bool alive = false;
    float4 rec0 = make_float4(0, 0, 0, 0), rec1 = rec0;
    float rgb2 = 0.f;
    uint32_t rect_lo = 0, rect_hi = 0;
    if (in_range) do {
        const f3 p = { a.means3D[3 * (size_t)i], a.means3D[3 * (size_t)i + 1], a.means3D[3 * (size_t)i + 2] };
        const f3 p_view = xform4x3(p, a.view);
        if (!a.prefiltered && p_view.z <= 0.01f) break;

        const float4 p_hom = xform4x4(p, a.proj);
        const float p_w = 1.0f / (p_hom.w + 0.0000001f);
        const float projx = p_hom.x * p_w, projy = p_hom.y * p_w;

        float cov3D[6];
        if (a.cov3D_precomp) {
#pragma unroll
            for (int q = 0; q < 6; q++) cov3D[q] = a.cov3D_precomp[6 * (size_t)i + q];
        } else if (a.g_indices) {
            const size_t g = (size_t)a.g_indices[i];
            const float4 rot = a.gtab[2 * g], sc = a.gtab[2 * g + 1];
            cov3d_from_scale_rot(sc.x, sc.y, sc.z, a.scale_factors[i] * a.scale_modifier, rot, cov3D);
        } else {
            const float4 rot = *reinterpret_cast<const float4*>(a.rotations + 4 * (size_t)i);
            cov3d_from_scale_rot(a.scales[3 * (size_t)i], a.scales[3 * (size_t)i + 1], a.scales[3 * (size_t)i + 2],
                                 a.scale_modifier, rot, cov3D);
        }
        const Cov2D cv = cov2d(p, a.focal_x, a.focal_y, a.tan_fovx, a.tan_fovy, cov3D, a.view);

        const float det = (cv.a * cv.c - cv.b * cv.b);
        if (det == 0.0f) break;
        const float det_inv = 1.f / det;
        const float conic_a = cv.c * det_inv, conic_b = -cv.b * det_inv, conic_c = cv.a * det_inv;

        const float mid = 0.5f * (cv.a + cv.c);
        const float lambda1 = mid + sqrtf(fmaxf(0.1f, mid * mid - det));
        const float lambda2 = mid - sqrtf(fmaxf(0.1f, mid * mid - det));
        const float my_radius = ceilf(3.f * sqrtf(fmaxf(lambda1, lambda2)));
        const float pix = ndc2pix(projx, a.W), piy = ndc2pix(projy, a.H);
        int x0, y0, x1, y1;
        get_rect(pix, piy, (int)my_radius, a.gx, a.gy, x0, y0, x1, y1);
        if ((x1 - x0) * (y1 - y0) == 0) break;

        float rgb[3];
        uint8_t clamp_bits = 0;
        if (a.colors_precomp) {
            rgb[0] = a.colors_precomp[3 * (size_t)i];
            rgb[1] = a.colors_precomp[3 * (size_t)i + 1];
            rgb[2] = a.colors_precomp[3 * (size_t)i + 2];
        } else {
            const size_t row = a.sh_indices ? (size_t)a.sh_indices[i] : (size_t)i;
            const float* shp = a.sh + row * (size_t)a.M * 3;
            constexpr int NC = (DEG + 1) * (DEG + 1) * 3;
            float c[NC];
            if ((a.M * 3) % 4 == 0 && NC % 4 == 0) {
#pragma unroll
                for (int q = 0; q < NC / 4; q++) {
                    const float4 v = reinterpret_cast<const float4*>(shp)[q];
                    c[4 * q] = v.x; c[4 * q + 1] = v.y; c[4 * q + 2] = v.z; c[4 * q + 3] = v.w;
                }
            } else {
#pragma unroll
                for (int q = 0; q < NC; q++) c[q] = shp[q];
            }
            f3 dir = { p.x - a.campos[0], p.y - a.campos[1], p.z - a.campos[2] };
            const float len = sqrtf(dir.x * dir.x + dir.y * dir.y + dir.z * dir.z);
            dir.x = dir.x / len; dir.y = dir.y / len; dir.z = dir.z / len;
            sh_to_rgb<DEG>(c, dir.x, dir.y, dir.z, rgb);
            if (a.clamp_color) {
#pragma unroll
                for (int ch = 0; ch < 3; ch++) {
                    if (rgb[ch] < 0) clamp_bits |= (uint8_t)(1u << ch);
                    rgb[ch] = fmaxf(rgb[ch], 0.0f);
                }
            }
        }

        alive = true;
        out_radius = (int32_t)my_radius;
        out_tiles = (uint32_t)((y1 - y0) * (x1 - x0));
        out_key = __float_as_uint(p_view.z);
        a.clamped[i] = clamp_bits;
        uint16_t* rc = a.rects + 4 * (size_t)i;
        rc[0] = (uint16_t)x0; rc[1] = (uint16_t)y0; rc[2] = (uint16_t)x1; rc[3] = (uint16_t)y1;
        rec0 = make_float4(pix, piy, conic_a, conic_b);
        rec1 = make_float4(conic_c, a.opacities[i], rgb[0], rgb[1]);
        rgb2 = rgb[2];
        rect_lo = (uint32_t)x0 | ((uint32_t)y0 << 16);
        rect_hi = (uint32_t)x1 | ((uint32_t)y1 << 16);
    } while (false);

    uint32_t incl = out_tiles;
#pragma unroll
    for (int o = 1; o < 64; o <<= 1) { const uint32_t v = __shfl_up(incl, o); if (lane >= o) incl += v; }
    if (lane == 63) s_wsum[wave] = incl;
    __syncthreads();
    uint32_t woff = 0;
    for (int w = 0; w < wave; w++) woff += s_wsum[w];
    const uint32_t my_incl = woff + incl;
    if (t == 255) a.block_total[blockIdx.x] = my_incl;
    if (!in_range) return;
    if (!alive) *reinterpret_cast<uint2*>(a.rects + 4 * (size_t)i) = make_uint2(0u, 0u);
    if (alive) {
        float4* rec = a.splat + 3 * (size_t)i;
        rec[0] = rec0;
        rec[1] = rec1;
        rec[2] = make_float4(rgb2, __uint_as_float(my_incl - out_tiles), __uint_as_float(rect_lo), __uint_as_float(rect_hi));
    }
    a.inst_offset[i] = my_incl;
    a.radii[i] = out_radius;
    a.depth_keys[i] = out_key;
}

__global__ void __launch_bounds__(1024) scan_blocks_kernel(int nb, uint32_t* __restrict__ base, const uint32_t* __restrict__ sort_err,
                                                           uint32_t* __restrict__ host_out, uint32_t host_seq)
{
    __shared__ uint32_t s_w[2][16];
    const int t = threadIdx.x, lane = t & 63, wave = t >> 6;
    uint32_t carry = 0;
    int buf = 0;
    for (int c0 = 0; c0 < nb; c0 += 16384, buf ^= 1) {
        const int i0 = c0 + t * 16;
        uint32_t v[16];
#pragma unroll
        for (int q = 0; q < 4; q++) {
            uint4 x = make_uint4(0u, 0u, 0u, 0u);
            if (i0 + 4 * q + 3 < nb) x = reinterpret_cast<const uint4*>(base + i0)[q];
            else {
                if (i0 + 4 * q < nb) x.x = base[i0 + 4 * q];
                if (i0 + 4 * q + 1 < nb) x.y = base[i0 + 4 * q + 1];
                if (i0 + 4 * q + 2 < nb) x.z = base[i0 + 4 * q + 2];
            }
            v[4 * q] = x.x; v[4 * q + 1] = x.y; v[4 * q + 2] = x.z; v[4 * q + 3] = x.w;
        }
        uint32_t mine = 0;
#pragma unroll
        for (int q = 0; q < 16; q++) mine += v[q];
        uint32_t incl = mine;
#pragma unroll
        for (int o = 1; o < 64; o <<= 1) { const uint32_t u = __shfl_up(incl, o); if (lane >= o) incl += u; }
        if (lane == 63) s_w[buf][wave] = incl;
        __syncthreads();
        uint32_t off = carry, all = 0;
#pragma unroll
        for (int w = 0; w < 16; w++) { const uint32_t x = s_w[buf][w]; if (w < wave) off += x; all += x; }
        uint32_t run = off + incl - mine;
#pragma unroll
        for (int q = 0; q < 16; q++) { const uint32_t x = v[q]; v[q] = run; run += x; }
#pragma unroll
        for (int q = 0; q < 4; q++) {
            if (i0 + 4 * q + 3 < nb) reinterpret_cast<uint4*>(base + i0)[q] = make_uint4(v[4 * q], v[4 * q + 1], v[4 * q + 2], v[4 * q + 3]);
            else {
                if (i0 + 4 * q < nb) base[i0 + 4 * q] = v[4 * q];
                if (i0 + 4 * q + 1 < nb) base[i0 + 4 * q + 1] = v[4 * q + 1];
                if (i0 + 4 * q + 2 < nb) base[i0 + 4 * q + 2] = v[4 * q + 2];
            }
        }
        carry += all;
    }
    __syncthreads();
    if (t == 0) {
        base[nb] = carry;
        const uint32_t err = sort_err ? *sort_err : 0u;
        if (sort_err) base[nb + 1] = err;
        if (host_out) {
            __hip_atomic_store(host_out, carry, __ATOMIC_RELAXED, __HIP_MEMORY_SCOPE_SYSTEM);
            __hip_atomic_store(host_out + 1, err, __ATOMIC_RELAXED, __HIP_MEMORY_SCOPE_SYSTEM);
            __hip_atomic_store(host_out + 2, host_seq, __ATOMIC_RELEASE, __HIP_MEMORY_SCOPE_SYSTEM);
        }
    }
}

void launch_preprocess(const c3dgs_raster_params& p, const GeomPtrs& g, int32_t* radii, uint2* ranges, const uint32_t* sort_err,
                       void* zero_span, size_t zero_n16, uint32_t* host_out, uint32_t host_seq, hipStream_t s)
{
    if (p.P <= 0) return;
    PreArgs a;
    a.P = p.P; a.M = p.M; a.W = p.W; a.H = p.H; a.gx = tiles_x(p.W); a.gy = tiles_y(p.H);
    a.means3D = p.means3D; a.sh = p.sh; a.colors_precomp = p.colors_precomp; a.opacities = p.opacities;
    a.scales = p.scales; a.scale_factors = p.scale_factors; a.rotations = p.rotations; a.cov3D_precomp = p.cov3D_precomp;
    a.sh_indices = p.sh_indices; a.g_indices = p.g_indices;
    a.view = p.viewmatrix; a.proj = p.projmatrix; a.campos = p.campos;
    a.tan_fovx = p.tan_fovx; a.tan_fovy = p.tan_fovy;
    a.focal_y = p.H / (2.0f * p.tan_fovy);
    a.focal_x = p.W / (2.0f * p.tan_fovx);
    a.scale_modifier = p.scale_modifier; a.prefiltered = p.prefiltered; a.clamp_color = p.clamp_color;
    a.radii = radii; a.splat = g.splat; a.rects = g.rects;
    a.clamped = g.clamped; a.depth_keys = g.depth_keys;
    a.inst_offset = g.inst_offset;
    a.block_total = g.block_base;
    a.ranges = ranges; a.T = a.gx * a.gy;
    a.gtab = g.gtab;
    a.zero_span = (uint4*)zero_span; a.zero_n16 = zero_span ? zero_n16 : 0;
    const dim3 grid((p.P + 255) / 256), block(256);
    const int deg = p.colors_precomp ? 0 : p.D;
    switch (deg) {
        case 0: preprocess_kernel<0><<<grid, block, 0, s>>>(a); break;
        case 1: preprocess_kernel<1><<<grid, block, 0, s>>>(a); break;
        case 2: preprocess_kernel<2><<<grid, block, 0, s>>>(a); break;
        default: preprocess_kernel<3><<<grid, block, 0, s>>>(a); break;
    }
    scan_blocks_kernel<<<1, 1024, 0, s>>>((int)grid.x, g.block_base, sort_err, host_out, host_seq);
}

__device__ __forceinline__ uint32_t rect_tiles(const uint2 rc)
{
    return (uint32_t)(((int)(rc.y & 0xffff) - (int)(rc.x & 0xffff)) * ((int)(rc.y >> 16) - (int)(rc.x >> 16)));
}

__global__ void __launch_bounds__(256)
block_totals_kernel(int n, const uint2* __restrict__ rects_sorted, uint32_t* __restrict__ totals)
{
    __shared__ uint32_t s_w[4];
    const int i = blockIdx.x * 256 + threadIdx.x;
    uint32_t x = i < n ? rect_tiles(rects_sorted[i]) : 0u;
#pragma unroll
    for (int o = 32; o > 0; o >>= 1) x += __shfl_xor(x, o);
    if ((threadIdx.x & 63) == 0) s_w[threadIdx.x >> 6] = x;
    __syncthreads();
    if (threadIdx.x == 0) totals[blockIdx.x] = (s_w[0] + s_w[1]) + (s_w[2] + s_w[3]);
}

template <class K>
__global__ void __launch_bounds__(256)
duplicate_with_keys_kernel(int P, const uint32_t* __restrict__ order, const uint2* __restrict__ rects_sorted,
                           const uint32_t* __restrict__ depth_base, K* __restrict__ keys, uint32_t* __restrict__ values,
                           int grid_x, const uint32_t* __restrict__ sort_err, uint4* __restrict__ zero_span, size_t zero_n16)
{
    if (zero_n16) {
        const size_t per = (zero_n16 + gridDim.x - 1) / gridDim.x, z0 = (size_t)blockIdx.x * per, z1 = min(z0 + per, zero_n16);
        for (size_t q = z0 + threadIdx.x; q < z1; q += 256) zero_span[q] = make_uint4(0u, 0u, 0u, 0u);
    }
    if (*sort_err) return;
    __shared__ uint32_t s_end[256];
    __shared__ uint32_t s_id[256];
    __shared__ uint2 s_rect[256];
    __shared__ uint32_t s_inv[256];
    __shared__ uint32_t s_wsum[4];
    const int t = threadIdx.x, lane = t & 63, wave = t >> 6;
    const int k0 = blockIdx.x * 256, k = k0 + t;
    const uint32_t out_begin = depth_base[blockIdx.x];
    uint32_t incl = 0;
    if (k < P) {
        const uint2 rc = rects_sorted[k];
        incl = rect_tiles(rc);
        s_id[t] = order[k];
        s_rect[t] = rc;
        const uint32_t w = (rc.y & 0xffff) - (rc.x & 0xffff);
        s_inv[t] = w > 1 ? 0xffffffffu / w + 1u : 0u;
    }
#pragma unroll
    for (int o = 1; o < 64; o <<= 1) { const uint32_t v = __shfl_up(incl, o); if (lane >= o) incl += v; }
    if (lane == 63) s_wsum[wave] = incl;
    __syncthreads();
    uint32_t woff = out_begin;
    for (int w = 0; w < wave; w++) woff += s_wsum[w];
    s_end[t] = woff + incl;
    __syncthreads();
    const int nk = min(256, P - k0);
    const uint32_t out_end = s_end[nk - 1];
    constexpr int CH = 1024;
    __shared__ uint16_t s_head[CH];
    __shared__ uint32_t s_wmax[4];
    const uint32_t my_tiles = k < P ? rect_tiles(s_rect[t]) : 0u;
    const uint32_t my_begin = s_end[t] - my_tiles;
    uint32_t carry = 0;
    for (uint32_t c0 = out_begin & ~3u; c0 < out_end; c0 += CH) {
        reinterpret_cast<uint2*>(s_head)[t] = make_uint2(0u, 0u);
        __syncthreads();
        if (my_tiles && my_begin >= c0 && my_begin < c0 + CH) s_head[my_begin - c0] = (uint16_t)(t + 1);
        __syncthreads();
        const uint2 hv = reinterpret_cast<const uint2*>(s_head)[t];
        uint32_t m[4] = { hv.x & 0xffffu, hv.x >> 16, hv.y & 0xffffu, hv.y >> 16 };
        m[1] = max(m[0], m[1]); m[2] = max(m[1], m[2]); m[3] = max(m[2], m[3]);
        uint32_t scan = m[3];
#pragma unroll
        for (int o = 1; o < 64; o <<= 1) { const uint32_t v = __shfl_up(scan, o); if (lane >= o) scan = max(scan, v); }
        uint32_t before = __shfl_up(scan, 1);
        if (lane == 0) before = 0;
        if (lane == 63) s_wmax[wave] = scan;
        __syncthreads();
        before = max(before, carry);
        for (int w = 0; w < wave; w++) before = max(before, s_wmax[w]);
        carry = max(max(carry, max(s_wmax[0], s_wmax[1])), max(s_wmax[2], s_wmax[3]));
        const uint32_t o0 = c0 + 4u * t;
        K kq[4];
        uint32_t vq[4];
#pragma unroll
        for (int e = 0; e < 4; e++) {
            const uint32_t o = o0 + e;
            const uint32_t own = max(before, m[e]);
            kq[e] = 0; vq[e] = 0;
            if (o >= out_begin && o < out_end) {
                const int g = (int)own - 1;
                const uint32_t first = (g == 0) ? out_begin : s_end[g - 1];
                const uint2 rc = s_rect[g];
                const int x0 = rc.x & 0xffff, y0 = rc.x >> 16, x1 = rc.y & 0xffff;
                const uint32_t local = o - first, w = (uint32_t)(x1 - x0), inv = s_inv[g];
                const uint32_t ry = inv ? __umulhi(local, inv) : local, rx = local - ry * w;
                kq[e] = (K)((y0 + ry) * grid_x + (x0 + rx));
                vq[e] = s_id[g];
            }
        }
        if (o0 >= out_begin && o0 + 4 <= out_end) {
            if constexpr (sizeof(K) == 2)
                *reinterpret_cast<uint2*>(keys + o0) = make_uint2((uint32_t)kq[0] | ((uint32_t)kq[1] << 16), (uint32_t)kq[2] | ((uint32_t)kq[3] << 16));
            else
                *reinterpret_cast<uint4*>(keys + o0) = make_uint4((uint32_t)kq[0], (uint32_t)kq[1], (uint32_t)kq[2], (uint32_t)kq[3]);
            *reinterpret_cast<uint4*>(values + o0) = make_uint4(vq[0], vq[1], vq[2], vq[3]);
        } else {
#pragma unroll
            for (int e = 0; e < 4; e++)
                if (o0 + e >= out_begin && o0 + e < out_end) { keys[o0 + e] = kq[e]; values[o0 + e] = vq[e]; }
        }
        __syncthreads();
    }
}

void launch_depth_order_scan(int P, const GeomPtrs& g, hipStream_t s)
{
    if (P <= 0) return;
    const int nb = (P + 255) / 256;
    block_totals_kernel<<<nb, 256, 0, s>>>(P, g.sorted_offsets, g.depth_base);
    scan_blocks_kernel<<<1, 1024, 0, s>>>(nb, g.depth_base, nullptr, nullptr, 0u);
}

void launch_duplicate_with_keys(int P, const GeomPtrs& g, const BinPtrs& b, int grid_x, const uint32_t* sort_err,
                                void* zero_span, size_t zero_n16, hipStream_t s)
{
    if (P <= 0) return;
    if (!zero_span) zero_n16 = 0;
    if (b.key_bytes == 4)
        duplicate_with_keys_kernel<uint32_t><<<(P + 255) / 256, 256, 0, s>>>(P, g.depth_order, g.sorted_offsets, g.depth_base,
                                                                             (uint32_t*)b.keys_unsorted, b.values_unsorted, grid_x, sort_err, (uint4*)zero_span, zero_n16);
    else
        duplicate_with_keys_kernel<uint16_t><<<(P + 255) / 256, 256, 0, s>>>(P, g.depth_order, g.sorted_offsets, g.depth_base,
                                                                             (uint16_t*)b.keys_unsorted, b.values_unsorted, grid_x, sort_err, (uint4*)zero_span, zero_n16);
}

template <class K>
__global__ void __launch_bounds__(256)
identify_ranges_kernel(int L, const K* __restrict__ keys, uint2* __restrict__ ranges, const uint32_t* __restrict__ sort_err)
{
    if (*sort_err) return;
    const int j = blockIdx.x * 256 + threadIdx.x;
    const int i0 = j * 8;
    if (i0 >= L) return;
    uint32_t cur8[8];
    if constexpr (sizeof(K) == 2) {
        const uint4 v = reinterpret_cast<const uint4*>(keys)[j];
        const uint32_t w[4] = { v.x, v.y, v.z, v.w };
#pragma unroll
        for (int e = 0; e < 8; e++) cur8[e] = (e & 1) ? (w[e >> 1] >> 16) : (w[e >> 1] & 0xffffu);
    } else {
        const uint4 v0 = reinterpret_cast<const uint4*>(keys)[2 * j], v1 = reinterpret_cast<const uint4*>(keys)[2 * j + 1];
        cur8[0] = v0.x; cur8[1] = v0.y; cur8[2] = v0.z; cur8[3] = v0.w; cur8[4] = v1.x; cur8[5] = v1.y; cur8[6] = v1.z; cur8[7] = v1.w;
    }
    uint32_t prev = i0 > 0 ? (uint32_t)keys[i0 - 1] : 0xffffffffu;
#pragma unroll
    for (int e = 0; e < 8; e++) {
        const int idx = i0 + e;
        if (idx < L) {
            const uint32_t cur = cur8[e];
            if (cur != prev) {
                if (idx > 0) ranges[prev].y = (uint32_t)idx;
                ranges[cur].x = (uint32_t)idx;
            }
            if (idx == L - 1) ranges[cur].y = (uint32_t)L;
            prev = cur;
        }
    }
}

void launch_identify_ranges(int R, const void* keys_sorted, int key_bytes, uint2* ranges, const uint32_t* sort_err, hipStream_t s)
{
    if (R <= 0) return;
    const int threads = (R + 7) / 8;
    if (key_bytes == 4) identify_ranges_kernel<uint32_t><<<(threads + 255) / 256, 256, 0, s>>>(R, (const uint32_t*)keys_sorted, ranges, sort_err);
    else identify_ranges_kernel<uint16_t><<<(threads + 255) / 256, 256, 0, s>>>(R, (const uint16_t*)keys_sorted, ranges, sort_err);
}

}
```

c3dgs_amd/csrc/radix_sort.hip:

```cpp
#include "common.hpp"
#include <algorithm>
#include <cstdlib>

namespace c3dgs {

constexpr int OS_RADIX = 256;
#ifndef C3DGS_OS_TILE32
#define C3DGS_OS_TILE32 12288
#endif
#ifndef C3DGS_OS_BLOCK32
#define C3DGS_OS_BLOCK32 512
#endif
constexpr int OS_TILE16 = 8192, OS_BLOCK16 = 1024;
template <class K> struct OsShape {
    static constexpr int TILE = sizeof(K) == 2 ? OS_TILE16 : C3DGS_OS_TILE32;
    static constexpr int BLOCK = sizeof(K) == 2 ? OS_BLOCK16 : C3DGS_OS_BLOCK32;
    static constexpr int IPT = TILE / BLOCK;
};
constexpr uint32_t OS_FLAG_AGG = 1u << 30, OS_FLAG_PRE = 2u << 30, OS_CNT_MASK = (1u << 30) - 1;
constexpr int OS_MAX_PASSES = 4;
#ifndef C3DGS_OS_SPIN_LIMIT
#define C3DGS_OS_SPIN_LIMIT (1u << 22)
#endif
constexpr uint32_t OS_SPIN_LIMIT = C3DGS_OS_SPIN_LIMIT;
__device__ uint32_t g_os_error;
#ifdef C3DGS_DIAG
__device__ unsigned long long g_os_times[64 * 8];
#endif
#ifdef C3DGS_OS_TIMING
#define OS_T(slot) if (tid == 0 && (bid & 3) == 0 && (bid >> 2) < 64) g_os_times[(bid >> 2) * 8 + (slot)] = __builtin_readcyclecounter();
#define OS_T_DRAIN() asm volatile("s_waitcnt vmcnt(0)");
#define OS_T_LOADS_DONE()                                                                                    \
    if (key[0] == (K)0x12345678 && val[OS_IPT - 1] == 0x87654321u) kout[0] = key[OS_IPT - 1];                \
    OS_T_DRAIN()
#else
#define OS_T(slot)
#define OS_T_DRAIN()
#define OS_T_LOADS_DONE()
#endif

struct OsPlan { int passes; int bits[OS_MAX_PASSES]; };

static OsPlan os_plan(int total_bits)
{
    OsPlan p;
    p.passes = (total_bits + 7) / 8;
    if (p.passes < 1) p.passes = 1;
    int left = total_bits < 1 ? 1 : total_bits;
    for (int i = 0; i < p.passes; i++) {
        const int b = (left + (p.passes - i) - 1) / (p.passes - i);
        p.bits[i] = b;
        left -= b;
    }
    return p;
}

template <class K> static size_t os_blocks(size_t n) { return (n + OsShape<K>::TILE - 1) / OsShape<K>::TILE; }
template <class K> constexpr bool os_pre_pass0() { return sizeof(K) == 2; }
constexpr int OS_TABLE_ROW = 2 * OS_RADIX;
template <class K> static size_t os_table_words(size_t n) { return os_pre_pass0<K>() ? os_blocks<K>(n) * OS_TABLE_ROW : 0; }
template <class K> static size_t os_ctrl_bytes(size_t n, int passes)
{
    return align_up(((size_t)passes * OS_RADIX + (size_t)passes * os_blocks<K>(n) * OS_RADIX + 64 + os_table_words<K>(n)) * sizeof(uint32_t));
}

constexpr int OS_HIST_BLOCK = 1024;
template <class K>
__global__ void __launch_bounds__(OS_HIST_BLOCK) os_hist_kernel(const K* __restrict__ keys, size_t n, OsPlan plan, uint32_t* __restrict__ hist)
{
    __shared__ uint32_t s_h[OS_MAX_PASSES][OS_RADIX];
    for (int q = threadIdx.x; q < OS_MAX_PASSES * OS_RADIX; q += OS_HIST_BLOCK) (&s_h[0][0])[q] = 0;
    __syncthreads();
    constexpr int VEC = 16 / sizeof(K);
    const size_t nvec = n / VEC;
    const uint4* k4 = reinterpret_cast<const uint4*>(keys);
    auto add = [&](uint32_t k) {
        int shift = 0;
        for (int p = 0; p < plan.passes; p++) {
            atomicAdd(&s_h[p][(k >> shift) & ((1u << plan.bits[p]) - 1u)], 1u);
            shift += plan.bits[p];
        }
    };
    auto add4 = [&](const uint4 v) {
        const uint32_t w[4] = { v.x, v.y, v.z, v.w };
#pragma unroll
        for (int e = 0; e < 4; e++) {
            if (sizeof(K) == 4) add(w[e]);
            else { add(w[e] & 0xffffu); add(w[e] >> 16); }
        }
    };
    const size_t stride = (size_t)gridDim.x * OS_HIST_BLOCK;
    size_t i = (size_t)blockIdx.x * OS_HIST_BLOCK + threadIdx.x;
    for (; i + 3 * stride < nvec; i += 4 * stride) {
        const uint4 v0 = k4[i], v1 = k4[i + stride], v2 = k4[i + 2 * stride], v3 = k4[i + 3 * stride];
        add4(v0); add4(v1); add4(v2); add4(v3);
    }
    for (; i < nvec; i += stride) add4(k4[i]);
    for (size_t j = nvec * VEC + (size_t)blockIdx.x * OS_HIST_BLOCK + threadIdx.x; j < n; j += stride) add((uint32_t)keys[j]);
    __syncthreads();
    for (int q = threadIdx.x; q < plan.passes * OS_RADIX; q += OS_HIST_BLOCK) {
        const uint32_t v = (&s_h[0][0])[q];
        if (v) atomicAdd(&hist[q], v);
    }
}

__global__ void __launch_bounds__(1024) os_tile_hist_kernel(const uint16_t* __restrict__ keys, uint32_t n, OsPlan plan, uint32_t* __restrict__ table)
{
    constexpr int TILE = OsShape<uint16_t>::TILE;
    static_assert(TILE == 8 * 1024, "one 16-byte load of 8 keys per thread");
    __shared__ uint32_t s_h[OS_TABLE_ROW];
    if (threadIdx.x < OS_TABLE_ROW) s_h[threadIdx.x] = 0;
    __syncthreads();
    const uint32_t base = blockIdx.x * (uint32_t)TILE + threadIdx.x * 8u;
    const uint32_t m0 = (1u << plan.bits[0]) - 1u, m1 = plan.passes > 1 ? (1u << plan.bits[1]) - 1u : 0u;
    auto add = [&](uint32_t k) {
        atomicAdd(&s_h[k & m0], 1u);
        if (plan.passes > 1) atomicAdd(&s_h[OS_RADIX + ((k >> plan.bits[0]) & m1)], 1u);
    };
    if (base + 8 <= n && (reinterpret_cast<uintptr_t>(keys) & 15u) == 0) {
        const uint4 v = *reinterpret_cast<const uint4*>(keys + base);
        const uint32_t w[4] = { v.x, v.y, v.z, v.w };
#pragma unroll
        for (int e = 0; e < 4; e++) { add(w[e] & 0xffffu); add(w[e] >> 16); }
    } else {
        for (uint32_t i = base; i < min(base + 8u, n); i++) add((uint32_t)keys[i]);
    }
    __syncthreads();
    const int t = threadIdx.x;
    if (t < OS_TABLE_ROW && (t >> 8) < plan.passes && (t & (OS_RADIX - 1)) < (1 << plan.bits[(t >> 8) & 1]))
        table[(size_t)t * gridDim.x + blockIdx.x] = s_h[t];
}

__global__ void __launch_bounds__(256) os_table_scan_kernel(uint32_t* __restrict__ table, uint32_t blocks, OsPlan plan, uint32_t* __restrict__ hist)
{
    __shared__ uint32_t s_w[4];
    const int n0 = 1 << plan.bits[0];
    const int pass = (int)blockIdx.x < n0 ? 0 : 1, digit = (int)blockIdx.x - (pass ? n0 : 0), col = pass * OS_RADIX + digit;
    uint32_t* column = table + (size_t)col * blocks;
    const int lane = threadIdx.x & 63, wave = threadIdx.x >> 6;
    uint32_t carry = 0;
    for (uint32_t b0 = 0; b0 < blocks; b0 += 256) {
        const uint32_t b = b0 + threadIdx.x;
        const uint32_t c = b < blocks ? column[b] : 0u;
        uint32_t incl = c;
#pragma unroll
        for (int o = 1; o < 64; o <<= 1) { const uint32_t t = __shfl_up(incl, o); if (lane >= o) incl += t; }
        __syncthreads();
        if (lane == 63) s_w[wave] = incl;
        __syncthreads();
        uint32_t off = carry;
        for (int w = 0; w < wave; w++) off += s_w[w];
        if (pass == 0 && b < blocks) column[b] = off + incl - c;
        carry += s_w[0] + s_w[1] + s_w[2] + s_w[3];
    }
    if (threadIdx.x == 0) hist[col] = carry;
}

__device__ __forceinline__ uint32_t os_load(const uint32_t* p) { return __hip_atomic_load(p, __ATOMIC_RELAXED, __HIP_MEMORY_SCOPE_AGENT); }
__device__ __forceinline__ void os_store(uint32_t* p, uint32_t v) { __hip_atomic_store(p, v, __ATOMIC_RELAXED, __HIP_MEMORY_SCOPE_AGENT); }

__device__ __forceinline__ uint32_t os_pack_rect(uint2 r)
{
    return (r.x & 0xffu) | ((r.x >> 16) << 8) | ((r.y & 0xffu) << 16) | ((r.y >> 16) << 24);
}
__device__ __forceinline__ uint2 os_unpack_rect(uint32_t w)
{
    return make_uint2((w & 0xffu) | (((w >> 8) & 0xffu) << 16), ((w >> 16) & 0xffu) | ((w >> 24) << 16));
}

template <class K, int BITS, bool PRE, bool PAY2 = false>
__global__ void __launch_bounds__(OsShape<K>::BLOCK)
os_pass_kernel(const K* __restrict__ kin, K* __restrict__ kout, const uint32_t* __restrict__ vin, uint32_t* __restrict__ vout,
               uint32_t n, int shift, const uint32_t* __restrict__ hist, uint32_t* __restrict__ status, uint32_t* __restrict__ ticket,
               const uint2* __restrict__ gather_src, uint2* __restrict__ gather_dst, const uint32_t* __restrict__ p2in = nullptr,
               uint32_t* __restrict__ p2out = nullptr)
{
    constexpr uint32_t ERR_BIT = sizeof(K) == 2 ? 1u : 2u;
    constexpr uint32_t MASK = (1u << BITS) - 1;
    constexpr int OS_BLOCK = OsShape<K>::BLOCK, OS_IPT = OsShape<K>::IPT, OS_WAVES = OS_BLOCK / 64;
    __shared__ uint32_t s_cnt[OS_WAVES][OS_RADIX];
    __shared__ uint32_t s_start[OS_RADIX];
    __shared__ int32_t s_gbase[OS_RADIX];
    __shared__ uint32_t s_wtot[4];
    __shared__ uint32_t s_bid;
    constexpr int OS_TILE = OsShape<K>::TILE;
    __shared__ K s_keys[OS_TILE];
    __shared__ uint32_t s_vals[OS_TILE];
    __shared__ uint32_t s_vals2[PAY2 ? OS_TILE : 1];

    const int tid = threadIdx.x, lane = tid & 63, wave = tid >> 6;
    if (tid == 0) s_bid = PRE ? blockIdx.x : atomicAdd(ticket, 1u);
    for (int q = tid; q < OS_WAVES * OS_RADIX; q += OS_BLOCK) (&s_cnt[0][0])[q] = 0;
    __syncthreads();
    const uint32_t bid = s_bid;
    OS_T(0)
    const uint32_t block_start = bid * (uint32_t)OS_TILE;
    const uint32_t valid = min((uint32_t)OS_TILE, n - block_start);

    K key[OS_IPT];
    uint32_t val[OS_IPT], rank[OS_IPT];
    uint32_t val2[PAY2 ? OS_IPT : 1];
    const uint32_t wbase = block_start + (uint32_t)wave * 64u * OS_IPT;
#pragma unroll
    for (int k = 0; k < OS_IPT; k++) {
        const uint32_t idx = wbase + (uint32_t)k * 64u + lane;
        const bool ok = idx < n;
        key[k] = ok ? kin[idx] : (K)0;
        val[k] = ok ? (vin ? vin[idx] : idx) : 0u;
        if (PAY2) val2[k] = ok ? (p2in ? p2in[idx] : os_pack_rect(gather_src[idx])) : 0u;
    }
    const uint32_t lt_lo = lane < 32 ? (1u << lane) - 1u : 0xffffffffu, lt_hi = lane < 32 ? 0u : (1u << (lane - 32)) - 1u;
    OS_T_LOADS_DONE()
    OS_T(1)
    uint32_t* wc = s_cnt[wave];
#pragma unroll
    for (int k = 0; k < OS_IPT; k++) {
        const uint32_t idx = wbase + (uint32_t)k * 64u + lane;
        const bool ok = idx < n;
        const uint32_t d = ((uint32_t)key[k] >> shift) & MASK;
        const unsigned long long okb = __ballot(ok);
        uint32_t plo = (uint32_t)okb, phi = (uint32_t)(okb >> 32);
#pragma unroll
        for (int b = 0; b < BITS; b++) {
            const int sgn = __builtin_amdgcn_sbfe((int)d, b, 1);
            const unsigned long long bal = __ballot(sgn != 0);
            plo &= ~((uint32_t)bal ^ (uint32_t)sgn);
            phi &= ~((uint32_t)(bal >> 32) ^ (uint32_t)sgn);
        }
        rank[k] = 0;
        if (ok) {
            const uint32_t before = __hip_atomic_load(&wc[d], __ATOMIC_RELAXED, __HIP_MEMORY_SCOPE_WAVEFRONT);
            const uint32_t below = (uint32_t)__popc(plo & lt_lo) + (uint32_t)__popc(phi & lt_hi);
            rank[k] = before + below;
            if (below == 0) __hip_atomic_store(&wc[d], before + (uint32_t)__popc(plo) + (uint32_t)__popc(phi), __ATOMIC_RELAXED, __HIP_MEMORY_SCOPE_WAVEFRONT);
        }
        __builtin_amdgcn_fence(__ATOMIC_RELEASE, "wavefront");
        __builtin_amdgcn_wave_barrier();
        __builtin_amdgcn_fence(__ATOMIC_ACQUIRE, "wavefront");
    }
    OS_T(2)
    __syncthreads();
    OS_T(3)
    uint32_t tot = 0;
    if (tid < OS_RADIX) {
#pragma unroll
        for (int w = 0; w < OS_WAVES; w++) { const uint32_t c = s_cnt[w][tid]; s_cnt[w][tid] = tot; tot += c; }
    }
    uint32_t incl = tot;
#pragma unroll
    for (int o = 1; o < 64; o <<= 1) { const uint32_t t = __shfl_up(incl, o); if (lane >= o) incl += t; }
    if (tid < OS_RADIX && lane == 63) s_wtot[wave] = incl;
    __syncthreads();
    uint32_t start = 0, pre = 0;
    if (tid < OS_RADIX) {
        uint32_t off = 0;
        for (int w = 0; w < wave; w++) off += s_wtot[w];
        start = off + incl - tot;
        s_start[tid] = start;
        uint32_t* my = status + (size_t)bid * OS_RADIX + tid;
        if (PRE) pre = tid < (1 << BITS) ? status[(size_t)tid * gridDim.x + bid] : 0u;
        else if (bid == 0) os_store(my, OS_FLAG_PRE | tot);
        else {
            os_store(my, OS_FLAG_AGG | tot);
            for (int64_t b = (int64_t)bid - 1;; b--) {
                uint32_t s, spins = 0;
                do { s = os_load(status + (size_t)b * OS_RADIX + tid); } while ((s >> 30) == 0 && ++spins < OS_SPIN_LIMIT);
                if ((s >> 30) == 0) { atomicOr(&g_os_error, ERR_BIT); break; }
                pre += s & OS_CNT_MASK;
                if (s & OS_FLAG_PRE) break;
            }
            os_store(my, OS_FLAG_PRE | (pre + tot));
        }
    }
    OS_T(4)
    const uint32_t h = tid < OS_RADIX ? hist[tid] : 0u;
    uint32_t hincl = h;
#pragma unroll
    for (int o = 1; o < 64; o <<= 1) { const uint32_t t = __shfl_up(hincl, o); if (lane >= o) hincl += t; }
    __syncthreads();
    if (tid < OS_RADIX && lane == 63) s_wtot[wave] = hincl;
    __syncthreads();
    if (tid < OS_RADIX) {
        uint32_t off = 0;
        for (int w = 0; w < wave; w++) off += s_wtot[w];
        s_gbase[tid] = (int32_t)(off + hincl - h + pre) - (int32_t)start;
    }
    OS_T(5)
#pragma unroll
    for (int k = 0; k < OS_IPT; k++) {
        const uint32_t idx = wbase + (uint32_t)k * 64u + lane;
        if (idx < n) {
            const uint32_t d = ((uint32_t)key[k] >> shift) & MASK;
            const uint32_t p = s_start[d] + s_cnt[wave][d] + rank[k];
            s_keys[p] = key[k];
            s_vals[p] = val[k];
            if (PAY2) s_vals2[p] = val2[k];
        }
    }
    __syncthreads();
    OS_T(6)
#pragma unroll
    for (int m = 0; m < OS_IPT; m++) {
        const uint32_t p = (uint32_t)tid + (uint32_t)m * OS_BLOCK;
        if (p < valid) {
            const K kk = s_keys[p];
            const uint32_t d = ((uint32_t)kk >> shift) & MASK;
            const uint32_t g = (uint32_t)(s_gbase[d] + (int32_t)p);
            kout[g] = kk;
            const uint32_t vv = s_vals[p];
            vout[g] = vv;
            if (PAY2) {
                if (p2out) p2out[g] = s_vals2[p];
                else gather_dst[g] = os_unpack_rect(s_vals2[p]);
            } else if (gather_src) gather_dst[g] = gather_src[vv];
        }
    }
    OS_T_DRAIN()
    OS_T(7)
}

template <class K, bool PRE>
static void os_launch_pass(int bits, unsigned blocks, hipStream_t s, const K* ki, K* ko, const uint32_t* vi, uint32_t* vo, uint32_t n,
                           int shift, const uint32_t* hist, uint32_t* status, uint32_t* ticket, const uint2* gsrc, uint2* gdst)
{
#define C3DGS_OS_CASE(B) case B: os_pass_kernel<K, B, PRE><<<blocks, OsShape<K>::BLOCK, 0, s>>>(ki, ko, vi, vo, n, shift, hist, status, ticket, gsrc, gdst); break
    switch (bits) {
        C3DGS_OS_CASE(1); C3DGS_OS_CASE(2); C3DGS_OS_CASE(3); C3DGS_OS_CASE(4);
        C3DGS_OS_CASE(5); C3DGS_OS_CASE(6); C3DGS_OS_CASE(7);
        default: os_pass_kernel<K, 8, PRE><<<blocks, OsShape<K>::BLOCK, 0, s>>>(ki, ko, vi, vo, n, shift, hist, status, ticket, gsrc, gdst); break;
    }
#undef C3DGS_OS_CASE
}

template <class K>
static size_t os_temp_bytes(size_t n, int total_bits, bool pay2 = false)
{
    const OsPlan plan = os_plan(total_bits);
    size_t b = os_ctrl_bytes<K>(n, plan.passes);
    const int bufs = plan.passes >= 3 ? 2 : (plan.passes == 2 ? 1 : 0);
    b += (size_t)bufs * (align_up(n * sizeof(K)) + align_up(n * sizeof(uint32_t)));
    if (pay2) b += 2 * align_up(n * sizeof(uint32_t));
    return b;
}

template <class K>
static size_t os_clear_bytes(size_t n, int total_bits)
{
    const OsPlan plan = os_plan(total_bits);
    if (!os_pre_pass0<K>()) return os_ctrl_bytes<K>(n, plan.passes);
    return ((size_t)plan.passes * OS_RADIX + (size_t)plan.passes * os_blocks<K>(n) * OS_RADIX + 64) * sizeof(uint32_t);
}

template <class K>
static hipError_t os_sort(void* temp, size_t temp_bytes, const K* kin, K* kout, const uint32_t* vin, uint32_t* vout, size_t n,
                          int total_bits, hipStream_t s, const uint2* gather_src = nullptr, uint2* gather_dst = nullptr,
                          bool ctrl_cleared = false, bool pay2 = false)
{
    if (n == 0) return hipSuccess;
    if (pay2 && (sizeof(K) != 4 || total_bits != 32 || !gather_src || !gather_dst || vin || os_temp_bytes<K>(n, total_bits, true) > temp_bytes))
        pay2 = false;
    if (n >= ((size_t)1 << 30) || os_temp_bytes<K>(n, total_bits) > temp_bytes) return hipErrorInvalidValue;
    const OsPlan plan = os_plan(total_bits);
    if (os_pre_pass0<K>() && plan.passes > 2) return hipErrorInvalidValue;
    const size_t blocks = os_blocks<K>(n);
    char* base = (char*)temp;
    const size_t ctrl = os_ctrl_bytes<K>(n, plan.passes);
    uint32_t* hist = (uint32_t*)base;
    uint32_t* status = hist + (size_t)plan.passes * OS_RADIX;
    uint32_t* ticket = status + (size_t)plan.passes * blocks * OS_RADIX;
    uint32_t* table = ticket + 64;
    constexpr bool pre0 = os_pre_pass0<K>();
    K* tk[2]; uint32_t* tv[2];
    char* q = base + ctrl;
    for (int i = 0; i < 2; i++) { tk[i] = (K*)q; q += align_up(n * sizeof(K)); tv[i] = (uint32_t*)q; q += align_up(n * sizeof(uint32_t)); }
    uint32_t* t2[2] = { nullptr, nullptr };
    if (pay2) {
        q = base + os_temp_bytes<K>(n, total_bits);
        for (int i = 0; i < 2; i++) { t2[i] = (uint32_t*)q; q += align_up(n * sizeof(uint32_t)); }
    }
    if (!ctrl_cleared) {
        const hipError_t e = hipMemsetAsync(base, 0, os_clear_bytes<K>(n, total_bits), s);
        if (e != hipSuccess) return e;
    }
    if constexpr (pre0) {
        os_tile_hist_kernel<<<(unsigned)blocks, 1024, 0, s>>>((const uint16_t*)kin, (uint32_t)n, plan, table);
        os_table_scan_kernel<<<(unsigned)((1 << plan.bits[0]) + (plan.passes > 1 ? (1 << plan.bits[1]) : 0)), 256, 0, s>>>(table, (uint32_t)blocks, plan, hist);
    } else {
        const size_t nvec16 = n * sizeof(K) / 16 + 1;
        const unsigned hb = (unsigned)std::min<size_t>((nvec16 + OS_HIST_BLOCK * 4 - 1) / (OS_HIST_BLOCK * 4), 512);
        os_hist_kernel<K><<<hb, OS_HIST_BLOCK, 0, s>>>(kin, n, plan, hist);
    }
    int shift = 0;
    for (int p = 0; p < plan.passes; p++) {
        const K* ki = p == 0 ? kin : tk[(p - 1) & 1];
        const uint32_t* vi = p == 0 ? vin : tv[(p - 1) & 1];
        K* ko = p == plan.passes - 1 ? kout : tk[p & 1];
        uint32_t* vo = p == plan.passes - 1 ? vout : tv[p & 1];
        const bool last = p == plan.passes - 1;
        if constexpr (sizeof(K) == 4) {
            if (pay2) {
                os_pass_kernel<K, 8, false, true><<<(unsigned)blocks, OsShape<K>::BLOCK, 0, s>>>(
                    ki, ko, vi, vo, (uint32_t)n, shift, hist + (size_t)p * OS_RADIX, status + (size_t)p * blocks * OS_RADIX, ticket + p,
                    gather_src, gather_dst, p == 0 ? nullptr : t2[(p - 1) & 1], last ? nullptr : t2[p & 1]);
                shift += plan.bits[p];
                continue;
            }
        }
        if (pre0 && p == 0)
            os_launch_pass<K, true>(plan.bits[p], (unsigned)blocks, s, ki, ko, vi, vo, (uint32_t)n, shift, hist, table, ticket,
                                    last ? gather_src : nullptr, last ? gather_dst : nullptr);
        else
            os_launch_pass<K, false>(plan.bits[p], (unsigned)blocks, s, ki, ko, vi, vo, (uint32_t)n, shift, hist + (size_t)p * OS_RADIX,
                                     status + (size_t)p * blocks * OS_RADIX, ticket + p, last ? gather_src : nullptr, last ? gather_dst : nullptr);
        shift += plan.bits[p];
    }
    return hipGetLastError();
}

#ifdef C3DGS_DIAG
int os_read_times(unsigned long long* out512)
{
    return hipMemcpyFromSymbol(out512, HIP_SYMBOL(g_os_times), sizeof(unsigned long long) * 512) != hipSuccess;
}
#endif

uint32_t* onesweep_error_word()
{
    static uint32_t* cache[64] = { nullptr };
    int dev = 0;
    if (hipGetDevice(&dev) != hipSuccess || dev < 0 || dev >= 64) return nullptr;
    if (!cache[dev]) {
        void* p = nullptr;
        if (hipGetSymbolAddress(&p, HIP_SYMBOL(g_os_error)) != hipSuccess) return nullptr;
        cache[dev] = (uint32_t*)p;
    }
    return cache[dev];
}

int onesweep_timed_out(hipStream_t s)
{
    if (!onesweep_enabled()) return 0;
    uint32_t* e = onesweep_error_word();
    uint32_t w = 1;
    if (!e || hipMemcpyAsync(&w, e, sizeof(w), hipMemcpyDeviceToHost, s) != hipSuccess) return 1;
    if (hipStreamSynchronize(s) != hipSuccess) return 1;
    if (w) (void)hipMemsetAsync(e, 0, sizeof(w), s);
    return w != 0;
}

bool onesweep_enabled()
{
    static const bool on = []() { const char* e = std::getenv("C3DGS_SORT_ROCPRIM"); return !(e && e[0] == '1'); }();
    return on;
}
size_t onesweep_depth_temp_bytes(int P) { return os_temp_bytes<uint32_t>((size_t)(P > 0 ? P : 1), 32, true); }
size_t onesweep_tile_temp_bytes(int R, int end_bit, int key_bytes)
{
    return key_bytes == 4 ? os_temp_bytes<uint32_t>((size_t)(R > 0 ? R : 1), end_bit) : os_temp_bytes<uint16_t>((size_t)(R > 0 ? R : 1), end_bit);
}
size_t onesweep_depth_clear_bytes(int P) { return os_clear_bytes<uint32_t>((size_t)(P > 0 ? P : 1), 32); }
size_t onesweep_tile_clear_bytes(int R, int end_bit, int key_bytes)
{
    return key_bytes == 4 ? os_clear_bytes<uint32_t>((size_t)(R > 0 ? R : 1), end_bit) : os_clear_bytes<uint16_t>((size_t)(R > 0 ? R : 1), end_bit);
}
hipError_t onesweep_tile_sort32(void* temp, size_t temp_bytes, const uint32_t* kin, uint32_t* kout, const uint32_t* vin, uint32_t* vout,
                                int R, int end_bit, hipStream_t s, bool ctrl_cleared)
{
    return os_sort<uint32_t>(temp, temp_bytes, kin, kout, vin, vout, (size_t)R, end_bit, s, nullptr, nullptr, ctrl_cleared);
}
hipError_t onesweep_depth_sort(void* temp, size_t temp_bytes, const uint32_t* kin, uint32_t* kout, const uint32_t* vin, uint32_t* vout,
                               int P, const uint2* gather_src, uint2* gather_dst, hipStream_t s, bool ctrl_cleared, bool rects_fit_bytes)
{
    static const bool no_pay2 = []() { const char* e = std::getenv("C3DGS_DEPTH_SORT_GATHER"); return e && e[0] == '1'; }();
    return os_sort<uint32_t>(temp, temp_bytes, kin, kout, vin, vout, (size_t)P, 32, s, gather_src, gather_dst, ctrl_cleared,
                             rects_fit_bytes && !no_pay2);
}
hipError_t onesweep_tile_sort(void* temp, size_t temp_bytes, const uint16_t* kin, uint16_t* kout, const uint32_t* vin, uint32_t* vout,
                              int R, int end_bit, hipStream_t s, bool ctrl_cleared)
{
    return os_sort<uint16_t>(temp, temp_bytes, kin, kout, vin, vout, (size_t)R, end_bit, s, nullptr, nullptr, ctrl_cleared);
}

}
```

Before: 622.4 views/s.

## Make onesweep radix passes persistent and fold depth block totals into sort

Converts the onesweep radix pass kernel into a persistent loop: the grid is capped at the resident block count and each block pulls further tiles from a ticket counter while overlapping the next tile's loads. The last depth-sort pass now also writes the per-256 block tile totals, so the separate block_totals kernel is skipped and the totals buffer is zeroed by preprocess. Launch bounds now carry a waves-per-SIMD hint. This removes launch and tail overhead and one kernel over P rects, at the cost of more kernel complexity, register pressure and a reliance on the ticket ordering for look-back.

```diff
diff --git a/__graft_entry__.py b/__graft_entry__.py
--- a/__graft_entry__.py
+++ b/__graft_entry__.py
@@ -11,7 +11,7 @@
     from c3dgs_amd import build as hip_build
     lib = hip_build.build()
     assert os.path.exists(lib)
-    for variant in hip_build.VARIANTS:
+    for variant in list(hip_build.VARIANTS) + list(hip_build.MORE_VARIANTS):
         assert os.path.exists(hip_build.build_variant(variant))
     subprocess.check_call(["make", "-C", os.path.join(ROOT, "oracle"), "-s"])
     import c3dgs_amd
diff --git a/c3dgs_amd/build.py b/c3dgs_amd/build.py
--- a/c3dgs_amd/build.py
+++ b/c3dgs_amd/build.py
@@ -52,6 +52,7 @@
 
 
 VARIANTS = {"spin1": {"radix_sort.hip": ["-DC3DGS_OS_SPIN_LIMIT=1u"]}}
+MORE_VARIANTS = {"grid3": {"radix_sort.hip": ["-DC3DGS_OS_PERSIST_GRID=3"]}}
 def _diag(mode):
     return {src: ["-DC3DGS_DIAG", mode] for src in ("render.hip", "radix_sort.hip", "diag.hip")}
 
@@ -61,7 +62,7 @@
 
 def build_variant(name, verbose=False):
     build(verbose=verbose)
-    flags = {**VARIANTS, **DIAG_VARIANTS}[name]
+    flags = {**VARIANTS, **MORE_VARIANTS, **DIAG_VARIANTS}[name]
     odir = os.path.join(HERE, "build", "variant_" + name)
     os.makedirs(odir, exist_ok=True)
     lib = os.path.join(HERE, f"libc3dgs_hip_{name}.so")
@@ -105,6 +106,6 @@
 
 if __name__ == "__main__":
     print(build(force="--force" in sys.argv, verbose="--verbose" in sys.argv or "-v" in sys.argv))
-    for flag, table in (("--variants", VARIANTS), ("--diag", DIAG_VARIANTS)):
+    for flag, table in (("--variants", {**VARIANTS, **MORE_VARIANTS}), ("--diag", DIAG_VARIANTS)):
         for v in table if flag in sys.argv else ():
             print(build_variant(v, verbose="--verbose" in sys.argv or "-v" in sys.argv))
diff --git a/c3dgs_amd/csrc/binning.hip b/c3dgs_amd/csrc/binning.hip
--- a/c3dgs_amd/csrc/binning.hip
+++ b/c3dgs_amd/csrc/binning.hip
@@ -49,10 +49,11 @@
 
 hipError_t run_depth_sort(void* temp, size_t temp_bytes, const uint32_t* kin, uint32_t* kout, const uint32_t* vin,
                           uint32_t* vout, int P, const uint2* rects, uint2* rects_sorted, hipStream_t s, bool ctrl_cleared,
-                          bool rects_fit_bytes)
+                          bool rects_fit_bytes, uint32_t* totals)
 {
     if (onesweep_enabled() && (size_t)P < ((size_t)1 << 30))
-        return onesweep_depth_sort(temp, temp_bytes, kin, kout, vin, vout, P, rects, rects_sorted, s, ctrl_cleared, rects_fit_bytes);
+        return onesweep_depth_sort(temp, temp_bytes, kin, kout, vin, vout, P, rects, rects_sorted, s, ctrl_cleared, rects_fit_bytes, totals);
+    if (totals) return hipErrorInvalidValue;
     hipError_t e = vin ? rocprim::radix_sort_pairs(temp, temp_bytes, kin, kout, vin, vout, (size_t)P, 0u, 32u, s)
                        : rocprim::radix_sort_pairs(temp, temp_bytes, kin, kout, rocprim::counting_iterator<uint32_t>(0u), vout,
                                                    (size_t)P, 0u, 32u, s);
diff --git a/c3dgs_amd/csrc/c_abi.hip b/c3dgs_amd/csrc/c_abi.hip
--- a/c3dgs_amd/csrc/c_abi.hip
+++ b/c3dgs_amd/csrc/c_abi.hip
@@ -200,19 +200,22 @@
     if (!hr.pinned) return fail(C3DGS_E_HIP, "pinned host buffer allocation failed");
     const uint32_t host_seq = hr.begin();
     const size_t dclear = depth_sort_clear_bytes(P) <= g.scan_temp_bytes ? depth_sort_clear_bytes(P) : 0;
+    const bool fold_totals = dclear != 0;
+    const size_t dbase_bytes = (size_t)((char*)g.scan_temp - (char*)g.depth_base);
     { StageTimer t_(ST_PREPROCESS, s);
       if (geom_gtab_bytes(p)) launch_pack_codebook(p, g.gtab, s);
-      launch_preprocess(p, g, radii, img.ranges, sort_err, g.scan_temp, dclear / 16, hr.dev, host_seq, s); }
+      launch_preprocess(p, g, radii, img.ranges, sort_err, fold_totals ? (void*)g.depth_base : g.scan_temp,
+                        fold_totals ? (dbase_bytes + dclear) / 16 : 0, hr.dev, host_seq, s); }
     C3DGS_STAGE_CHECK(ST_PREPROCESS, p.debug, s);
     const uint32_t* r_words = g.block_base + (P + 255) / 256;
     if (int rc = hr.queue_copy(r_words, s)) return rc;
     { StageTimer t_(ST_DEPTH_SORT, s);
       C3DGS_HIP_TRY(run_depth_sort(g.scan_temp, g.scan_temp_bytes, g.depth_keys, g.depth_keys_sorted, nullptr, g.depth_order, P,
                                    reinterpret_cast<const uint2*>(g.rects), g.sorted_offsets, s, dclear != 0,
-                                   gx <= 255 && gy <= 255)); }
+                                   gx <= 255 && gy <= 255, fold_totals ? g.depth_base : nullptr)); }
     C3DGS_STAGE_CHECK(ST_DEPTH_SORT, p.debug, s);
     if (p.debug && onesweep_timed_out(s)) return fail(C3DGS_E_HIP, "depth sort: look-back timed out");
-    C3DGS_TIMED_STAGE(ST_SCAN, p.debug, s, launch_depth_order_scan(P, g, s));
+    C3DGS_TIMED_STAGE(ST_SCAN, p.debug, s, launch_depth_order_scan(P, g, fold_totals, s));
     uint32_t words[2];
     if (int rc = hr.wait(r_words, s, words)) return rc;
     const uint32_t R_u = words[0];
diff --git a/c3dgs_amd/csrc/common.hpp b/c3dgs_amd/csrc/common.hpp
--- a/c3dgs_amd/csrc/common.hpp
+++ b/c3dgs_amd/csrc/common.hpp
@@ -45,6 +45,11 @@
     float f;
     memcpy(&f, &u, 4);
     return f;
+}
+
+__device__ __forceinline__ uint32_t rect_tiles(const uint2 rc)
+{
+    return (uint32_t)(((int)(rc.y & 0xffff) - (int)(rc.x & 0xffff)) * ((int)(rc.y >> 16) - (int)(rc.x >> 16)));
 }
 
 inline size_t align_up(size_t v, size_t a = 256) { return (v + a - 1) / a * a; }
@@ -202,13 +207,13 @@
 void launch_pack_codebook(const c3dgs_raster_params& p, float4* gtab, hipStream_t s);
 void launch_preprocess(const c3dgs_raster_params& p, const GeomPtrs& g, int32_t* radii, uint2* ranges, const uint32_t* sort_err,
                        void* zero_span, size_t zero_n16, uint32_t* host_out, uint32_t host_seq, hipStream_t s);
-void launch_depth_order_scan(int P, const GeomPtrs& g, hipStream_t s);
+void launch_depth_order_scan(int P, const GeomPtrs& g, bool totals_done, hipStream_t s);
 void launch_duplicate_with_keys(int P, const GeomPtrs& g, const BinPtrs& b, int grid_x, const uint32_t* sort_err,
                                 void* zero_span, size_t zero_n16, hipStream_t s);
 void launch_identify_ranges(int R, const void* keys_sorted, int key_bytes, uint2* ranges, const uint32_t* sort_err, hipStream_t s);
 hipError_t run_depth_sort(void* temp, size_t temp_bytes, const uint32_t* kin, uint32_t* kout, const uint32_t* vin,
                           uint32_t* vout, int P, const uint2* rects, uint2* rects_sorted, hipStream_t s, bool ctrl_cleared = false,
-                          bool rects_fit_bytes = false);
+                          bool rects_fit_bytes = false, uint32_t* totals = nullptr);
 hipError_t run_tile_sort(void* temp, size_t temp_bytes, const void* kin, void* kout, int key_bytes, const uint32_t* vin,
                          uint32_t* vout, int R, int end_bit, hipStream_t s, bool ctrl_cleared = false);
 size_t depth_sort_clear_bytes(int P);
@@ -222,7 +227,7 @@
 size_t onesweep_tile_clear_bytes(int R, int end_bit, int key_bytes);
 hipError_t onesweep_depth_sort(void* temp, size_t temp_bytes, const uint32_t* kin, uint32_t* kout, const uint32_t* vin, uint32_t* vout,
                                int P, const uint2* gather_src, uint2* gather_dst, hipStream_t s, bool ctrl_cleared = false,
-                               bool rects_fit_bytes = false);
+                               bool rects_fit_bytes = false, uint32_t* totals = nullptr);
 hipError_t onesweep_tile_sort32(void* temp, size_t temp_bytes, const uint32_t* kin, uint32_t* kout, const uint32_t* vin, uint32_t* vout,
                                 int R, int end_bit, hipStream_t s, bool ctrl_cleared = false);
 hipError_t onesweep_tile_sort(void* temp, size_t temp_bytes, const uint16_t* kin, uint16_t* kout, const uint32_t* vin, uint32_t* vout,
diff --git a/c3dgs_amd/csrc/preprocess.hip b/c3dgs_amd/csrc/preprocess.hip
--- a/c3dgs_amd/csrc/preprocess.hip
+++ b/c3dgs_amd/csrc/preprocess.hip
@@ -363,11 +363,6 @@
     scan_blocks_kernel<<<1, 1024, 0, s>>>((int)grid.x, g.block_base, sort_err, host_out, host_seq);
 }
 
-__device__ __forceinline__ uint32_t rect_tiles(const uint2 rc)
-{
-    return (uint32_t)(((int)(rc.y & 0xffff) - (int)(rc.x & 0xffff)) * ((int)(rc.y >> 16) - (int)(rc.x >> 16)));
-}
-
 __global__ void __launch_bounds__(256)
 block_totals_kernel(int n, const uint2* __restrict__ rects_sorted, uint32_t* __restrict__ totals)
 {
@@ -477,11 +472,11 @@
     }
 }
 
-void launch_depth_order_scan(int P, const GeomPtrs& g, hipStream_t s)
+void launch_depth_order_scan(int P, const GeomPtrs& g, bool totals_done, hipStream_t s)
 {
     if (P <= 0) return;
     const int nb = (P + 255) / 256;
-    block_totals_kernel<<<nb, 256, 0, s>>>(P, g.sorted_offsets, g.depth_base);
+    if (!totals_done) block_totals_kernel<<<nb, 256, 0, s>>>(P, g.sorted_offsets, g.depth_base);
     scan_blocks_kernel<<<1, 1024, 0, s>>>(nb, g.depth_base, nullptr, nullptr, 0u);
 }
 
diff --git a/c3dgs_amd/csrc/radix_sort.hip b/c3dgs_amd/csrc/radix_sort.hip
--- a/c3dgs_amd/csrc/radix_sort.hip
+++ b/c3dgs_amd/csrc/radix_sort.hip
@@ -16,6 +16,7 @@
     static constexpr int TILE = sizeof(K) == 2 ? OS_TILE16 : C3DGS_OS_TILE32;
     static constexpr int BLOCK = sizeof(K) == 2 ? OS_BLOCK16 : C3DGS_OS_BLOCK32;
     static constexpr int IPT = TILE / BLOCK;
+    static constexpr int WAVES_PER_SIMD = sizeof(K) == 2 ? 8 : 2;
 };
 constexpr uint32_t OS_FLAG_AGG = 1u << 30, OS_FLAG_PRE = 2u << 30, OS_CNT_MASK = (1u << 30) - 1;
 constexpr int OS_MAX_PASSES = 4;
@@ -31,7 +32,7 @@
 #define OS_T(slot) if (tid == 0 && (bid & 3) == 0 && (bid >> 2) < 64) g_os_times[(bid >> 2) * 8 + (slot)] = __builtin_readcyclecounter();
 #define OS_T_DRAIN() asm volatile("s_waitcnt vmcnt(0)");
 #define OS_T_LOADS_DONE()                                                                                    \
-    if (key[0] == (K)0x12345678 && val[OS_IPT - 1] == 0x87654321u) kout[0] = key[OS_IPT - 1];                \
+    if (key[0] == 0x12345678u && val[OS_IPT - 1] == 0x87654321u) kout[0] = (K)key[OS_IPT - 1];                \
     OS_T_DRAIN()
 #else
 #define OS_T(slot)
@@ -169,15 +170,16 @@
 }
 
 template <class K, int BITS, bool PRE, bool PAY2 = false>
-__global__ void __launch_bounds__(OsShape<K>::BLOCK)
+__global__ void __launch_bounds__(OsShape<K>::BLOCK, OsShape<K>::WAVES_PER_SIMD)
 os_pass_kernel(const K* __restrict__ kin, K* __restrict__ kout, const uint32_t* __restrict__ vin, uint32_t* __restrict__ vout,
-               uint32_t n, int shift, const uint32_t* __restrict__ hist, uint32_t* __restrict__ status, uint32_t* __restrict__ ticket,
-               const uint2* __restrict__ gather_src, uint2* __restrict__ gather_dst, const uint32_t* __restrict__ p2in = nullptr,
-               uint32_t* __restrict__ p2out = nullptr)
+               uint32_t n, uint32_t tiles, int shift, const uint32_t* __restrict__ hist, uint32_t* __restrict__ status,
+               uint32_t* __restrict__ ticket, const uint2* __restrict__ gather_src, uint2* __restrict__ gather_dst,
+               const uint32_t* __restrict__ p2in = nullptr, uint32_t* __restrict__ p2out = nullptr, uint32_t* __restrict__ totals = nullptr)
 {
     constexpr uint32_t ERR_BIT = sizeof(K) == 2 ? 1u : 2u;
     constexpr uint32_t MASK = (1u << BITS) - 1;
     constexpr int OS_BLOCK = OsShape<K>::BLOCK, OS_IPT = OsShape<K>::IPT, OS_WAVES = OS_BLOCK / 64;
+    constexpr bool TOTALS = sizeof(K) == 4;
     __shared__ uint32_t s_cnt[OS_WAVES][OS_RADIX];
     __shared__ uint32_t s_start[OS_RADIX];
     __shared__ int32_t s_gbase[OS_RADIX];
@@ -190,144 +192,218 @@
 
     const int tid = threadIdx.x, lane = tid & 63, wave = tid >> 6;
     if (tid == 0) s_bid = PRE ? blockIdx.x : atomicAdd(ticket, 1u);
-    for (int q = tid; q < OS_WAVES * OS_RADIX; q += OS_BLOCK) (&s_cnt[0][0])[q] = 0;
-    __syncthreads();
-    const uint32_t bid = s_bid;
-    OS_T(0)
-    const uint32_t block_start = bid * (uint32_t)OS_TILE;
-    const uint32_t valid = min((uint32_t)OS_TILE, n - block_start);
-
-    K key[OS_IPT];
-    uint32_t val[OS_IPT], rank[OS_IPT];
-    uint32_t val2[PAY2 ? OS_IPT : 1];
-    const uint32_t wbase = block_start + (uint32_t)wave * 64u * OS_IPT;
-#pragma unroll
-    for (int k = 0; k < OS_IPT; k++) {
-        const uint32_t idx = wbase + (uint32_t)k * 64u + lane;
-        const bool ok = idx < n;
-        key[k] = ok ? kin[idx] : (K)0;
-        val[k] = ok ? (vin ? vin[idx] : idx) : 0u;
-        if (PAY2) val2[k] = ok ? (p2in ? p2in[idx] : os_pack_rect(gather_src[idx])) : 0u;
-    }
-    const uint32_t lt_lo = lane < 32 ? (1u << lane) - 1u : 0xffffffffu, lt_hi = lane < 32 ? 0u : (1u << (lane - 32)) - 1u;
-    OS_T_LOADS_DONE()
-    OS_T(1)
-    uint32_t* wc = s_cnt[wave];
-#pragma unroll
-    for (int k = 0; k < OS_IPT; k++) {
-        const uint32_t idx = wbase + (uint32_t)k * 64u + lane;
-        const bool ok = idx < n;
-        const uint32_t d = ((uint32_t)key[k] >> shift) & MASK;
-        const unsigned long long okb = __ballot(ok);
-        uint32_t plo = (uint32_t)okb, phi = (uint32_t)(okb >> 32);
-#pragma unroll
-        for (int b = 0; b < BITS; b++) {
-            const int sgn = __builtin_amdgcn_sbfe((int)d, b, 1);
-            const unsigned long long bal = __ballot(sgn != 0);
-            plo &= ~((uint32_t)bal ^ (uint32_t)sgn);
-            phi &= ~((uint32_t)(bal >> 32) ^ (uint32_t)sgn);
-        }
-        rank[k] = 0;
-        if (ok) {
-            const uint32_t before = __hip_atomic_load(&wc[d], __ATOMIC_RELAXED, __HIP_MEMORY_SCOPE_WAVEFRONT);
-            const uint32_t below = (uint32_t)__popc(plo & lt_lo) + (uint32_t)__popc(phi & lt_hi);
-            rank[k] = before + below;
-            if (below == 0) __hip_atomic_store(&wc[d], before + (uint32_t)__popc(plo) + (uint32_t)__popc(phi), __ATOMIC_RELAXED, __HIP_MEMORY_SCOPE_WAVEFRONT);
-        }
-        __builtin_amdgcn_fence(__ATOMIC_RELEASE, "wavefront");
-        __builtin_amdgcn_wave_barrier();
-        __builtin_amdgcn_fence(__ATOMIC_ACQUIRE, "wavefront");
-    }
-    OS_T(2)
-    __syncthreads();
-    OS_T(3)
-    uint32_t tot = 0;
-    if (tid < OS_RADIX) {
-#pragma unroll
-        for (int w = 0; w < OS_WAVES; w++) { const uint32_t c = s_cnt[w][tid]; s_cnt[w][tid] = tot; tot += c; }
-    }
-    uint32_t incl = tot;
-#pragma unroll
-    for (int o = 1; o < 64; o <<= 1) { const uint32_t t = __shfl_up(incl, o); if (lane >= o) incl += t; }
-    if (tid < OS_RADIX && lane == 63) s_wtot[wave] = incl;
-    __syncthreads();
-    uint32_t start = 0, pre = 0;
-    if (tid < OS_RADIX) {
-        uint32_t off = 0;
-        for (int w = 0; w < wave; w++) off += s_wtot[w];
-        start = off + incl - tot;
-        s_start[tid] = start;
-        uint32_t* my = status + (size_t)bid * OS_RADIX + tid;
-        if (PRE) pre = tid < (1 << BITS) ? status[(size_t)tid * gridDim.x + bid] : 0u;
-        else if (bid == 0) os_store(my, OS_FLAG_PRE | tot);
-        else {
-            os_store(my, OS_FLAG_AGG | tot);
-            for (int64_t b = (int64_t)bid - 1;; b--) {
-                uint32_t s, spins = 0;
-                do { s = os_load(status + (size_t)b * OS_RADIX + tid); } while ((s >> 30) == 0 && ++spins < OS_SPIN_LIMIT);
-                if ((s >> 30) == 0) { atomicOr(&g_os_error, ERR_BIT); break; }
-                pre += s & OS_CNT_MASK;
-                if (s & OS_FLAG_PRE) break;
-            }
-            os_store(my, OS_FLAG_PRE | (pre + tot));
-        }
-    }
-    OS_T(4)
     const uint32_t h = tid < OS_RADIX ? hist[tid] : 0u;
     uint32_t hincl = h;
 #pragma unroll
     for (int o = 1; o < 64; o <<= 1) { const uint32_t t = __shfl_up(hincl, o); if (lane >= o) hincl += t; }
-    __syncthreads();
     if (tid < OS_RADIX && lane == 63) s_wtot[wave] = hincl;
     __syncthreads();
+    uint32_t bid = s_bid;
+    if (bid >= tiles) return;
+    uint32_t hbase = 0;
     if (tid < OS_RADIX) {
-        uint32_t off = 0;
-        for (int w = 0; w < wave; w++) off += s_wtot[w];
-        s_gbase[tid] = (int32_t)(off + hincl - h + pre) - (int32_t)start;
-    }
-    OS_T(5)
-#pragma unroll
-    for (int k = 0; k < OS_IPT; k++) {
-        const uint32_t idx = wbase + (uint32_t)k * 64u + lane;
-        if (idx < n) {
-            const uint32_t d = ((uint32_t)key[k] >> shift) & MASK;
-            const uint32_t p = s_start[d] + s_cnt[wave][d] + rank[k];
-            s_keys[p] = key[k];
-            s_vals[p] = val[k];
-            if (PAY2) s_vals2[p] = val2[k];
-        }
-    }
-    __syncthreads();
-    OS_T(6)
-#pragma unroll
-    for (int m = 0; m < OS_IPT; m++) {
-        const uint32_t p = (uint32_t)tid + (uint32_t)m * OS_BLOCK;
-        if (p < valid) {
-            const K kk = s_keys[p];
-            const uint32_t d = ((uint32_t)kk >> shift) & MASK;
-            const uint32_t g = (uint32_t)(s_gbase[d] + (int32_t)p);
-            kout[g] = kk;
-            const uint32_t vv = s_vals[p];
-            vout[g] = vv;
-            if (PAY2) {
-                if (p2out) p2out[g] = s_vals2[p];
-                else gather_dst[g] = os_unpack_rect(s_vals2[p]);
-            } else if (gather_src) gather_dst[g] = gather_src[vv];
-        }
-    }
-    OS_T_DRAIN()
-    OS_T(7)
+        for (int w = 0; w < wave; w++) hbase += s_wtot[w];
+        hbase += hincl - h;
+    }
+
+    constexpr bool RANK_IN_KEY = sizeof(K) == 2;
+    uint32_t key[OS_IPT], val[OS_IPT], rank[RANK_IN_KEY ? 1 : OS_IPT];
+    uint32_t val2[PAY2 ? OS_IPT : 1];
+    auto load_tile = [&](uint32_t b) {
+        const uint32_t wb = b * (uint32_t)OS_TILE + (uint32_t)wave * 64u * OS_IPT + lane, last = n - 1u;
+#pragma unroll
+        for (int k = 0; k < OS_IPT; k++) key[k] = (uint32_t)kin[min(wb + (uint32_t)k * 64u, last)];
+        if (vin) {
+#pragma unroll
+            for (int k = 0; k < OS_IPT; k++) val[k] = vin[min(wb + (uint32_t)k * 64u, last)];
+        } else {
+#pragma unroll
+            for (int k = 0; k < OS_IPT; k++) val[k] = wb + (uint32_t)k * 64u;
+        }
+        if (PAY2) {
+            if (p2in) {
+#pragma unroll
+                for (int k = 0; k < OS_IPT; k++) val2[k] = p2in[min(wb + (uint32_t)k * 64u, last)];
+            } else {
+#pragma unroll
+                for (int k = 0; k < OS_IPT; k++) val2[k] = os_pack_rect(gather_src[min(wb + (uint32_t)k * 64u, last)]);
+            }
+        }
+    };
+    uint32_t* wc = s_cnt[wave];
+    uint32_t next = bid, valid = 0;
+    for ([[maybe_unused]] int trip = 0;; trip++) {
+        if (trip == 0) { OS_T(0) }
+        if (next < tiles) load_tile(next);
+#pragma unroll
+        for (int m = 0; m < OS_IPT; m++) {
+            const uint32_t p = (uint32_t)tid + (uint32_t)m * OS_BLOCK;
+            uint32_t seg = 0xffffffffu, area = 0;
+            if (p < valid) {
+                const K kk = s_keys[p];
+                const uint32_t d = ((uint32_t)kk >> shift) & MASK;
+                const uint32_t g = (uint32_t)(s_gbase[d] + (int32_t)p);
+                kout[g] = kk;
+                const uint32_t vv = s_vals[p];
+                vout[g] = vv;
+                if (PAY2) {
+                    if (p2out) p2out[g] = s_vals2[p];
+                    else {
+                        const uint2 rc = os_unpack_rect(s_vals2[p]);
+                        gather_dst[g] = rc;
+                        seg = g >> 8; area = rect_tiles(rc);
+                    }
+                } else if (gather_src) {
+                    const uint2 rc = gather_src[vv];
+                    gather_dst[g] = rc;
+                    seg = g >> 8; area = rect_tiles(rc);
+                }
+            }
+            if (TOTALS && totals) {
+#pragma unroll
+                for (int o = 1; o < 64; o <<= 1) {
+                    const uint32_t a = __shfl_up(area, o), sg = __shfl_up(seg, o);
+                    if (lane >= o && sg == seg) area += a;
+                }
+                const uint32_t after = __shfl_down(seg, 1);
+                if (seg != 0xffffffffu && area && (lane == 63 || after != seg)) atomicAdd(&totals[seg], area);
+            }
+        }
+        if (trip == 1) { OS_T_DRAIN() OS_T(7) }
+        if (next >= tiles) break;
+        bid = next;
+        for (int q = tid; q < OS_WAVES * OS_RADIX; q += OS_BLOCK) (&s_cnt[0][0])[q] = 0;
+        __syncthreads();
+        const uint32_t block_start = bid * (uint32_t)OS_TILE;
+        valid = min((uint32_t)OS_TILE, n - block_start);
+        const uint32_t wbase = block_start + (uint32_t)wave * 64u * OS_IPT;
+        if (trip == 0) { OS_T_LOADS_DONE() OS_T(1) }
+#pragma unroll
+        for (int k = 0; k < OS_IPT; k++) {
+            const uint32_t idx = wbase + (uint32_t)k * 64u + lane;
+            const bool ok = idx < n;
+            const uint32_t d = (key[k] >> shift) & MASK;
+            const unsigned long long okb = __ballot(ok);
+            uint32_t plo = (uint32_t)okb, phi = (uint32_t)(okb >> 32);
+#pragma unroll
+            for (int b = 0; b < BITS; b++) {
+                const int sgn = __builtin_amdgcn_sbfe((int)d, b, 1);
+                const unsigned long long bal = __ballot(sgn != 0);
+                plo &= ~((uint32_t)bal ^ (uint32_t)sgn);
+                phi &= ~((uint32_t)(bal >> 32) ^ (uint32_t)sgn);
+            }
+            uint32_t r = 0;
+            if (ok) {
+                const uint32_t before = __hip_atomic_load(&wc[d], __ATOMIC_RELAXED, __HIP_MEMORY_SCOPE_WAVEFRONT);
+                const uint32_t below = __builtin_amdgcn_mbcnt_hi(phi, __builtin_amdgcn_mbcnt_lo(plo, 0u));
+                r = before + below;
+                if (below == 0) __hip_atomic_store(&wc[d], before + (uint32_t)__popc(plo) + (uint32_t)__popc(phi), __ATOMIC_RELAXED, __HIP_MEMORY_SCOPE_WAVEFRONT);
+            }
+            if constexpr (RANK_IN_KEY) key[k] |= r << 16; else rank[k] = r;
+            __builtin_amdgcn_fence(__ATOMIC_RELEASE, "wavefront");
+            __builtin_amdgcn_wave_barrier();
+            __builtin_amdgcn_fence(__ATOMIC_ACQUIRE, "wavefront");
+        }
+        if (trip == 0) { OS_T(2) }
+        __syncthreads();
+        if (trip == 0) { OS_T(3) }
+        uint32_t tot = 0;
+        if (tid < OS_RADIX) {
+#pragma unroll
+            for (int w = 0; w < OS_WAVES; w++) { const uint32_t c = s_cnt[w][tid]; s_cnt[w][tid] = tot; tot += c; }
+        }
+        uint32_t incl = tot;
+#pragma unroll
+        for (int o = 1; o < 64; o <<= 1) { const uint32_t t = __shfl_up(incl, o); if (lane >= o) incl += t; }
+        if (tid < OS_RADIX && lane == 63) s_wtot[wave] = incl;
+        __syncthreads();
+        if (tid < OS_RADIX) {
+            uint32_t off = 0, pre = 0;
+            for (int w = 0; w < wave; w++) off += s_wtot[w];
+            const uint32_t start = off + incl - tot;
+            s_start[tid] = start;
+            uint32_t* my = status + (size_t)bid * OS_RADIX + tid;
+            if (PRE) pre = tid < (1 << BITS) ? status[(size_t)tid * tiles + bid] : 0u;
+            else if (bid == 0) os_store(my, OS_FLAG_PRE | tot);
+            else {
+                os_store(my, OS_FLAG_AGG | tot);
+                for (int64_t b = (int64_t)bid - 1;; b--) {
+                    uint32_t s, spins = 0;
+                    do { s = os_load(status + (size_t)b * OS_RADIX + tid); } while ((s >> 30) == 0 && ++spins < OS_SPIN_LIMIT);
+                    if ((s >> 30) == 0) { atomicOr(&g_os_error, ERR_BIT); break; }
+                    pre += s & OS_CNT_MASK;
+                    if (s & OS_FLAG_PRE) break;
+                }
+                os_store(my, OS_FLAG_PRE | (pre + tot));
+            }
+            if (trip == 0) { OS_T(4) }
+            s_gbase[tid] = (int32_t)(hbase + pre) - (int32_t)start;
+        } else if (!PRE && tid == OS_BLOCK - 64) {
+            s_bid = atomicAdd(ticket, 1u);
+        }
+        __syncthreads();
+        if (trip == 0) { OS_T(5) }
+#pragma unroll
+        for (int k = 0; k < OS_IPT; k++) {
+            const uint32_t idx = wbase + (uint32_t)k * 64u + lane;
+            if (idx < n) {
+                const uint32_t d = (key[k] >> shift) & MASK;
+                uint32_t r;
+                if constexpr (RANK_IN_KEY) r = key[k] >> 16; else r = rank[k];
+                const uint32_t p = s_start[d] + s_cnt[wave][d] + r;
+                s_keys[p] = (K)key[k];
+                s_vals[p] = val[k];
+                if (PAY2) s_vals2[p] = val2[k];
+            }
+        }
+        next = PRE ? bid + gridDim.x : s_bid;
+        __syncthreads();
+        if (trip == 0) { OS_T(6) }
+    }
+}
+
+template <class K, int BITS, bool PRE, bool PAY2>
+static unsigned os_grid(size_t tiles)
+{
+    static int resident[64];
+    int dev = 0;
+    if (hipGetDevice(&dev) != hipSuccess || dev < 0 || dev >= 64) return 0;
+    if (!resident[dev]) {
+        int per_cu = 0, cus = 0;
+        if (hipOccupancyMaxActiveBlocksPerMultiprocessor(&per_cu, os_pass_kernel<K, BITS, PRE, PAY2>, OsShape<K>::BLOCK, 0) != hipSuccess ||
+            hipDeviceGetAttribute(&cus, hipDeviceAttributeMultiprocessorCount, dev) != hipSuccess || per_cu < 1 || cus < 1)
+            return 0;
+        resident[dev] = per_cu * cus;
+    }
+    size_t g = std::min<size_t>(tiles, (size_t)resident[dev]);
+#ifdef C3DGS_OS_PERSIST_GRID
+    g = std::min<size_t>(g, C3DGS_OS_PERSIST_GRID);
+#endif
+    return (unsigned)g;
+}
+
+template <class K, int BITS, bool PRE, bool PAY2 = false>
+static hipError_t os_launch(unsigned tiles, hipStream_t s, const K* ki, K* ko, const uint32_t* vi, uint32_t* vo, uint32_t n, int shift,
+                            const uint32_t* hist, uint32_t* status, uint32_t* ticket, const uint2* gsrc, uint2* gdst,
+                            const uint32_t* p2in = nullptr, uint32_t* p2out = nullptr, uint32_t* totals = nullptr)
+{
+    const unsigned grid = os_grid<K, BITS, PRE, PAY2>(tiles);
+    if (!grid) return hipErrorInvalidConfiguration;
+    os_pass_kernel<K, BITS, PRE, PAY2><<<grid, OsShape<K>::BLOCK, 0, s>>>(ki, ko, vi, vo, n, tiles, shift, hist, status, ticket, gsrc, gdst,
+                                                                         p2in, p2out, totals);
+    return hipSuccess;
 }
 
 template <class K, bool PRE>
-static void os_launch_pass(int bits, unsigned blocks, hipStream_t s, const K* ki, K* ko, const uint32_t* vi, uint32_t* vo, uint32_t n,
-                           int shift, const uint32_t* hist, uint32_t* status, uint32_t* ticket, const uint2* gsrc, uint2* gdst)
-{
-#define C3DGS_OS_CASE(B) case B: os_pass_kernel<K, B, PRE><<<blocks, OsShape<K>::BLOCK, 0, s>>>(ki, ko, vi, vo, n, shift, hist, status, ticket, gsrc, gdst); break
+static hipError_t os_launch_pass(int bits, unsigned tiles, hipStream_t s, const K* ki, K* ko, const uint32_t* vi, uint32_t* vo, uint32_t n,
+                                 int shift, const uint32_t* hist, uint32_t* status, uint32_t* ticket, const uint2* gsrc, uint2* gdst,
+                                 uint32_t* totals)
+{
+#define C3DGS_OS_CASE(B) case B: return os_launch<K, B, PRE>(tiles, s, ki, ko, vi, vo, n, shift, hist, status, ticket, gsrc, gdst, nullptr, nullptr, totals)
     switch (bits) {
         C3DGS_OS_CASE(1); C3DGS_OS_CASE(2); C3DGS_OS_CASE(3); C3DGS_OS_CASE(4);
         C3DGS_OS_CASE(5); C3DGS_OS_CASE(6); C3DGS_OS_CASE(7);
-        default: os_pass_kernel<K, 8, PRE><<<blocks, OsShape<K>::BLOCK, 0, s>>>(ki, ko, vi, vo, n, shift, hist, status, ticket, gsrc, gdst); break;
+        default: return os_launch<K, 8, PRE>(tiles, s, ki, ko, vi, vo, n, shift, hist, status, ticket, gsrc, gdst, nullptr, nullptr, totals);
     }
 #undef C3DGS_OS_CASE
 }
@@ -354,7 +430,7 @@
 template <class K>
 static hipError_t os_sort(void* temp, size_t temp_bytes, const K* kin, K* kout, const uint32_t* vin, uint32_t* vout, size_t n,
                           int total_bits, hipStream_t s, const uint2* gather_src = nullptr, uint2* gather_dst = nullptr,
-                          bool ctrl_cleared = false, bool pay2 = false)
+                          bool ctrl_cleared = false, bool pay2 = false, uint32_t* totals = nullptr)
 {
     if (n == 0) return hipSuccess;
     if (pay2 && (sizeof(K) != 4 || total_bits != 32 || !gather_src || !gather_dst || vin || os_temp_bytes<K>(n, total_bits, true) > temp_bytes))
@@ -397,21 +473,26 @@
         K* ko = p == plan.passes - 1 ? kout : tk[p & 1];
         uint32_t* vo = p == plan.passes - 1 ? vout : tv[p & 1];
         const bool last = p == plan.passes - 1;
+        uint32_t* tot = last && gather_dst ? totals : nullptr;
+        hipError_t e;
         if constexpr (sizeof(K) == 4) {
             if (pay2) {
-                os_pass_kernel<K, 8, false, true><<<(unsigned)blocks, OsShape<K>::BLOCK, 0, s>>>(
-                    ki, ko, vi, vo, (uint32_t)n, shift, hist + (size_t)p * OS_RADIX, status + (size_t)p * blocks * OS_RADIX, ticket + p,
-                    gather_src, gather_dst, p == 0 ? nullptr : t2[(p - 1) & 1], last ? nullptr : t2[p & 1]);
+                e = os_launch<K, 8, false, true>((unsigned)blocks, s, ki, ko, vi, vo, (uint32_t)n, shift, hist + (size_t)p * OS_RADIX,
+                                                 status + (size_t)p * blocks * OS_RADIX, ticket + p, gather_src, gather_dst,
+                                                 p == 0 ? nullptr : t2[(p - 1) & 1], last ? nullptr : t2[p & 1], tot);
+                if (e != hipSuccess) return e;
                 shift += plan.bits[p];
                 continue;
             }
         }
         if (pre0 && p == 0)
-            os_launch_pass<K, true>(plan.bits[p], (unsigned)blocks, s, ki, ko, vi, vo, (uint32_t)n, shift, hist, table, ticket,
-                                    last ? gather_src : nullptr, last ? gather_dst : nullptr);
+            e = os_launch_pass<K, true>(plan.bits[p], (unsigned)blocks, s, ki, ko, vi, vo, (uint32_t)n, shift, hist, table, ticket,
+                                        last ? gather_src : nullptr, last ? gather_dst : nullptr, tot);
         else
-            os_launch_pass<K, false>(plan.bits[p], (unsigned)blocks, s, ki, ko, vi, vo, (uint32_t)n, shift, hist + (size_t)p * OS_RADIX,
-                                     status + (size_t)p * blocks * OS_RADIX, ticket + p, last ? gather_src : nullptr, last ? gather_dst : nullptr);
+            e = os_launch_pass<K, false>(plan.bits[p], (unsigned)blocks, s, ki, ko, vi, vo, (uint32_t)n, shift, hist + (size_t)p * OS_RADIX,
+                                         status + (size_t)p * blocks * OS_RADIX, ticket + p, last ? gather_src : nullptr,
+                                         last ? gather_dst : nullptr, tot);
+        if (e != hipSuccess) return e;
         shift += plan.bits[p];
     }
     return hipGetLastError();
@@ -469,11 +550,12 @@
     return os_sort<uint32_t>(temp, temp_bytes, kin, kout, vin, vout, (size_t)R, end_bit, s, nullptr, nullptr, ctrl_cleared);
 }
 hipError_t onesweep_depth_sort(void* temp, size_t temp_bytes, const uint32_t* kin, uint32_t* kout, const uint32_t* vin, uint32_t* vout,
-                               int P, const uint2* gather_src, uint2* gather_dst, hipStream_t s, bool ctrl_cleared, bool rects_fit_bytes)
+                               int P, const uint2* gather_src, uint2* gather_dst, hipStream_t s, bool ctrl_cleared, bool rects_fit_bytes,
+                               uint32_t* totals)
 {
     static const bool no_pay2 = []() { const char* e = std::getenv("C3DGS_DEPTH_SORT_GATHER"); return e && e[0] == '1'; }();
     return os_sort<uint32_t>(temp, temp_bytes, kin, kout, vin, vout, (size_t)P, 32, s, gather_src, gather_dst, ctrl_cleared,
-                             rects_fit_bytes && !no_pay2);
+                             rects_fit_bytes && !no_pay2, totals);
 }
 hipError_t onesweep_tile_sort(void* temp, size_t temp_bytes, const uint16_t* kin, uint16_t* kout, const uint32_t* vin, uint32_t* vout,
                               int R, int end_bit, hipStream_t s, bool ctrl_cleared)
```

Result: no change. 618.2 views/s (-0.7%).
